# Lymphatus/caesium-clt

Hardware: AMD Instinct MI355X
Metric: megapixels/sec JPEG q=80 1920x1080 batch (higher is better)
Workload: dtype int32

## Files before the change

caesium-clt_amd/binding.py:

```python
import ctypes as C
import os

_HERE = os.path.dirname(os.path.abspath(__file__))
NPHASES = 8
NKERNELS = 36
PHASE_NAMES = ["decode", "pixel", "masks_flags_runs", "stats_tables", "sizes_scan", "pack", "stuff_assemble", "reserved"]


class CCSParameters(C.Structure):
    _fields_ = [("keep_metadata", C.c_bool), ("jpeg_quality", C.c_uint32), ("jpeg_chroma_subsampling", C.c_uint32),
                ("jpeg_progressive", C.c_bool), ("jpeg_optimize", C.c_bool), ("jpeg_preserve_icc", C.c_bool),
                ("png_quality", C.c_uint32), ("png_optimization_level", C.c_uint32), ("png_force_zopfli", C.c_bool),
                ("png_optimize", C.c_bool), ("gif_quality", C.c_uint32), ("webp_quality", C.c_uint32), ("webp_lossless", C.c_bool),
                ("tiff_compression", C.c_uint32), ("tiff_deflate_level", C.c_uint32), ("width", C.c_uint32), ("height", C.c_uint32)]


class CCSResult(C.Structure):
    _fields_ = [("success", C.c_bool), ("code", C.c_uint32), ("error_message", C.c_char_p)]


class CByteArray(C.Structure):
    _fields_ = [("data", C.POINTER(C.c_uint8)), ("length", C.c_size_t)]


class Timing(C.Structure):
    _fields_ = [("total_ms", C.c_float), ("phase_ms", C.c_float * NPHASES), ("kernel_ms", C.c_float * NKERNELS), ("in_bytes", C.c_uint64), ("out_bytes", C.c_uint64),
                ("pixels", C.c_uint64), ("coef_bytes", C.c_uint64), ("n_images", C.c_uint32), ("n_failed", C.c_uint32), ("n_seq_decoded", C.c_uint32), ("n_par_fallback", C.c_uint32), ("n_par_short", C.c_uint32), ("n_prog_decoded", C.c_uint32), ("n_refine_chains", C.c_uint32), ("n_search_extra", C.c_uint32), ("n_fused_lists", C.c_uint32), ("n_list_refine", C.c_uint32)]


class PngTiming(C.Structure):
    _fields_ = [("total_ms", C.c_float), ("kernel_ms", C.c_float * 16), ("in_bytes", C.c_uint64), ("out_bytes", C.c_uint64), ("pixels", C.c_uint64),
                ("raw_bytes", C.c_uint64), ("n_images", C.c_uint32), ("n_failed", C.c_uint32), ("n_trials", C.c_uint32)]


class CaesiumError(RuntimeError):
    def __init__(self, code, message):
        super().__init__(f"[{code}] {message}")
        self.code = code


def library_path():
    return os.path.join(_HERE, "libcaesium_hip.so")


EXPORTS = ["cs_default_parameters", "cs_compress_in_memory", "cs_compress_to_size_in_memory", "cs_convert_in_memory",
           "cs_batch_compress", "cs_batch_extent", "cs_free_bytes", "cs_free_result", "csh_device_count", "csh_last_error", "csh_kernel_name", "csh_kernel_name_webp", "csh_release_cached_memory", "csh_warmup", "csh_batch_create",
           "csh_batch_run", "csh_batch_fetch", "csh_batch_destroy", "csh_batch_retain_dct", "csh_batch_set_quality", "csh_batch_rerun_encode", "cs_batch_compress_to_size", "csh_batch_geometry", "csh_batch_read_coefs",
           "csp_kernel_name", "csp_batch_create", "csp_batch_create_webp", "csp_batch_create_pixels", "csh_batch_create_pixels", "csh_batch_pixels", "csh_batch_create_from_pixels", "csp_png_to_jpeg", "csp_png_to_lossless_webp", "csp_batch_run", "csp_batch_fetch", "csp_batch_destroy", "csp_batch_geometry", "csp_batch_read_rows", "csp_batch_read_stream",
           "csp_batch_trials", "csp_batch_read_scores", "csp_batch_chunk_bits", "csh_batch_create_webp", "cs_batch_convert",
           "cswd_batch_create", "cswd_batch_run", "cswd_batch_pixels", "cswd_batch_read_pixels", "cswd_batch_alpha", "cswd_batch_read_rgba", "cswd_batch_destroy", "cswd_rgba_join", "cswd_rgba_destroy", "csh_batch_create_webp_from_pixels", "csh_batch_create_from_pixels_rgb", "csl_encode_pixels", "csl_attach_alpha"]


def _declare(L):
    P = C.POINTER
    L.cs_default_parameters.argtypes = [P(CCSParameters)]
    L.cs_default_parameters.restype = None
    L.cs_compress_in_memory.argtypes = [C.c_char_p, C.c_size_t, P(CCSParameters), P(CByteArray)]
    L.cs_compress_in_memory.restype = CCSResult
    L.cs_compress_to_size_in_memory.argtypes = [C.c_char_p, C.c_size_t, P(CCSParameters), C.c_size_t, C.c_bool, P(CByteArray)]
    L.cs_compress_to_size_in_memory.restype = CCSResult
    L.cs_convert_in_memory.argtypes = [C.c_char_p, C.c_size_t, P(CCSParameters), C.c_uint32, P(CByteArray)]
    L.cs_convert_in_memory.restype = CCSResult
    L.cs_batch_compress.argtypes = [P(CByteArray), C.c_size_t, P(CCSParameters), C.c_int, P(CByteArray), P(CCSResult)]
    L.cs_batch_extent.argtypes = [P(CByteArray), C.c_size_t]
    L.cs_batch_extent.restype = C.c_size_t
    L.cs_free_bytes.argtypes = [P(CByteArray)]
    L.cs_free_bytes.restype = None
    L.cs_free_result.argtypes = [P(CCSResult)]
    L.cs_free_result.restype = None
    L.csh_last_error.restype = C.c_char_p
    L.csh_kernel_name.argtypes = [C.c_int]
    L.csh_kernel_name.restype = C.c_char_p
    L.csh_kernel_name_webp.argtypes = [C.c_int]
    L.csh_kernel_name_webp.restype = C.c_char_p
    L.csh_batch_create.argtypes = [P(CByteArray), C.c_size_t, P(CCSParameters), C.c_int, P(C.c_void_p)]
    L.csh_batch_run.argtypes = [C.c_void_p, P(Timing)]
    L.csh_batch_fetch.argtypes = [C.c_void_p, P(CByteArray), P(CCSResult)]
    L.csh_batch_retain_dct.argtypes = [C.c_void_p, C.c_int]
    L.csh_batch_set_quality.argtypes = [C.c_void_p, P(C.c_uint32)]
    L.csh_batch_rerun_encode.argtypes = [C.c_void_p, P(Timing)]
# ... 374 lines not shown
```

caesium-clt_amd/csrc/batch.hpp:

```cpp
#pragma once
#include <array>
#include <chrono>
#include <map>
#include <string>
#include <vector>

#include "../../include/caesium_hip.h"
#include "devmem.hpp"
#include "jpeg_host.hpp"
#include "kernels.h"
#include "webp_kernels.h"

namespace csh {

struct Item {
    int code = 0;
    std::string msg;
    JpegInfo in;
    JpegInfo out;
    int image = -1;
    size_t file_size = 0;
    std::vector<uint8_t> meta_out;
};

// ... 40 lines not shown
    uint32_t max_row_in = 0, max_out_w = 0, max_nh = 0;
    uint32_t max_src_px = 0;
    uint64_t plane_bytes = 0, oplane_bytes = 0;
    uint32_t max_quads = 0;
    bool any_layout = false, any_layout_rgb = false;

    DevBuf<uint8_t> d_planes, d_oplanes, d_rgb;
    DevBuf<PlaneWork> d_pwork;
    DevBuf<ResizeWork> d_rwork;
    DevBuf<ResizeTap> d_rtaps;
    DevBuf<float> d_rweights, d_rtmp;
    DevBuf<int16_t> d_dct_raw;
};

struct Stage {
    uint32_t work0 = 0, nwork = 0, slot0 = 0, nslots = 0, ech0 = 0, nech = 0, table0 = 0, ntables = 0, plan0 = 0, nplans = 0, nzc0 = 0, nnzc = 0, ls0 = 0, nls = 0, ts0 = 0, nts = 0, rs0 = 0, nrs = 0;
    bool nz_build[2] = {true, true}, nz_filter[2] = {true, true};
};
struct SearchImg {
    int cand_work[64]; int ncand;
    int Al_luma = 0, Al_chroma = 0;
    uint64_t best_luma = 0, best_chroma = 0;
    int split_luma = 0, split_chroma = 0;
    bool luma_on = false, chroma_on = false;
};

struct EncodePlan {
    std::vector<EncScan> script;
    std::vector<ScanWork> swork;
    uint32_t nslots = 0, nlist_slots = 0, ntok_slots = 0;
    uint32_t nref_slots = 0;
    uint32_t last_run_refine = 0;
    uint64_t total_corr = 0;
    uint64_t total_units = 0, total_words = 0;
    uint32_t max_units = 0;
    int ntables = 0;
    std::vector<TokPlan> plans;
    std::vector<int> plan_comp, plan_image;
    std::vector<EChunk> echunks;
    uint64_t tok_cap = 0;
    uint32_t tok_scale = 1;
    std::vector<TokRegion> regions;
    std::vector<uint32_t> region_est;
    uint32_t hist_rows = 0;
    std::vector<NzList> nzlists;
    std::vector<NzSet> nzsets;
    std::vector<int> nzset_of;
    std::vector<uint32_t> nzset_built;
    std::vector<int> nzset_comp, nzset_image;
    std::vector<NzChunk> nzchunks;
    std::vector<NzChunk> nzchunks_fused;
    uint32_t n_fused = 0;
    uint32_t last_run_fused = 0;
    std::vector<uint32_t> nz_est, nz_worst;
    uint32_t nz_nrec = 0;
    uint64_t nz_cap = 0;
    bool search = false;
    enum { ST_1 = 0, ST_1B = 1, ST_2 = 2, ST_2B = 3, ST_2C = 4, ST_N = 5 };
    Stage stage[ST_N];
    void stage_begin(Stage &sg) {
        sg.work0 = uint32_t(swork.size()); sg.slot0 = nslots; sg.ech0 = uint32_t(echunks.size()); sg.table0 = uint32_t(ntables); sg.plan0 = uint32_t(plans.size());
        sg.nzc0 = uint32_t(nzchunks.size()); sg.ls0 = nlist_slots; sg.ts0 = ntok_slots; sg.rs0 = nref_slots;
    }
    void stage_end(Stage &sg) {
        sg.nwork = uint32_t(swork.size()) - sg.work0; sg.nslots = nslots - sg.slot0; sg.nech = uint32_t(echunks.size()) - sg.ech0;
        sg.ntables = uint32_t(ntables) - sg.table0; sg.nplans = uint32_t(plans.size()) - sg.plan0;
        sg.nnzc = uint32_t(nzchunks.size()) - sg.nzc0; sg.nls = nlist_slots - sg.ls0; sg.nts = ntok_slots - sg.ts0; sg.nrs = nref_slots - sg.rs0;
    }
    std::vector<SearchImg> simg;
    std::vector<uint8_t> work_active;
    uint32_t n_gated_runs = 0;
    std::vector<uint32_t> img_list, img_nlist, h_cost;
    std::map<std::array<int, 5>, int> cand_script;
    std::vector<uint8_t> hdr_pool;
    std::vector<uint32_t> hdr_off;

    DevBuf<uint8_t> d_hdr, d_tail, d_scan_tmp, d_work_active;
    DevBuf<EncScan> d_script;
    DevBuf<ScanWork> d_swork;
    DevBuf<uint32_t> d_slot_work;
    DevBuf<EChunk> d_echunks;
    DevBuf<SlotRec> d_slots;
    DevBuf<TokPlan> d_plans;
    DevBuf<uint64_t> d_corr, d_symbits, d_eobbits, d_tok_off, d_chunk_off, d_scan_raw_off;
    DevBuf<uint32_t> d_tok_cursor;
    DevBuf<TokRegion> d_regions;
    DevBuf<uint16_t> d_eobrun, d_slot_hist;
    DevBuf<uint32_t> d_img_list, d_img_nlist, d_scan_cost, d_slot_raw, d_slot_eobh, d_long_runs, d_long_cnt, d_tokens, d_chunk_ntok, d_chunk_bits, d_raw, d_scan_pad, d_chunk_ff, d_hdr_off;
    DevBuf<DevEncTable> d_tables;
    DevBuf<NzList> d_nzlists;
    DevBuf<NzSet> d_nzsets;
    DevBuf<NzChunk> d_nzchunks, d_nzchunks_fused;
    DevBuf<uint32_t> d_nz_pool, d_nz_cursor, d_nz_chunk_off, d_nz_chunk_cnt, d_list_slots, d_tok_slots, d_ref_slots;
};

struct TrellisPlan {
    bool trellis = false, dering = false;
    Stage tstage;
    std::vector<TrellisWork> twork;
    std::vector<TrellisRun> truns;
    uint32_t t_units = 0, t_max_rows = 0;
    std::vector<uint32_t> trows;
    bool t_sort = false;
    bool nz_once = false;

    DevBuf<TrellisWork> d_twork;
// ... 50 lines not shown
    uint32_t ntiles = 0, ntiles_in = 0, ntiles_out = 0, max_tiles = 0, max_dummy = 0;
    csh::DevBuf<csh::ImgDesc> d_imgs;
    csh::DevBuf<csh::DevQuant> d_quants;
    csh::DevBuf<int16_t> d_coef;

    csh::DecodePlan dec;
    csh::PixelPlan pix;
    csh::EncodePlan enc;
    csh::TrellisPlan tr;
    csh::WebpTail wp;
    csh::Outputs out;

    ~csh_batch() { if (have_stream) { (void)hipStreamSynchronize(stream); (void)hipStreamDestroy(stream); } }
};

namespace csh {

enum KernelSlot {
    KS_MEMSET_COEF, KS_UNSTUFF, KS_DEC_SPEC, KS_DEC_RELAX0, KS_DEC_RELAX, KS_DEC_WRITE, KS_DC_SCATTER, KS_REFINE_CHAINS, KS_DECODE_PROG_SEQ,
    KS_IDCT_PLANE, KS_RESIZE, KS_XFORM_DIRECT, KS_RESAMPLE_FDCT, KS_FIX_DUMMY, KS_MEMSET_ENC, KS_TRELLIS_STATS, KS_TRELLIS_AC, KS_TRELLIS_DC,
    KS_NZLIST, KS_TOKENS, KS_LIST_STATS, KS_AC_RUNS, KS_GEN_TABLES, KS_CHUNK_SIZES, KS_SCAN_CHUNK_BITS, KS_SCAN_LAYOUT, KS_PACK, KS_LIST_PACK,
    KS_FF_COUNT, KS_SCAN_SEARCH, KS_LAYOUT, KS_SCAN_IMAGES, KS_EMIT, KS_SPARE0, KS_SPARE1, KS_SPARE2, KS_COUNT,
    KS_WEBP_YUV = KS_XFORM_DIRECT, KS_WEBP_ENCODE = KS_RESAMPLE_FDCT, KS_WEBP_ASSEMBLE = KS_FIX_DUMMY
};
struct KernelSlotRow { KernelSlot slot; const char *name; int phase; };
constexpr KernelSlotRow kKernelSlots[] = {
    {KS_MEMSET_COEF, "memset_coef", 0},        {KS_UNSTUFF, "unstuff", 0},                 {KS_DEC_SPEC, "k_dec_spec", 0},
    {KS_DEC_RELAX0, "k_dec_relax0", 0},        {KS_DEC_RELAX, "k_dec_relax1_4", 0},        {KS_DEC_WRITE, "k_dec_write", 0},
    {KS_DC_SCATTER, "k_dc_scatter", 0},        {KS_REFINE_CHAINS, "k_refine_chains", 0},   {KS_DECODE_PROG_SEQ, "k_decode_prog+seq", 0},
    {KS_IDCT_PLANE, "k_idct_plane", 1},        {KS_RESIZE, "resize", 1},                   {KS_XFORM_DIRECT, "k_xform_direct", 1},
    {KS_RESAMPLE_FDCT, "k_resample+k_plane_fdct", 1}, {KS_FIX_DUMMY, "k_fix_dummy", 1},    {KS_MEMSET_ENC, "memset_enc", 2},
    {KS_TRELLIS_STATS, "trellis_stats", 1},    {KS_TRELLIS_AC, "k_trellis_ac", 1},         {KS_TRELLIS_DC, "k_trellis_dc", 1},
    {KS_NZLIST, "k_nzlist", 2},                {KS_TOKENS, "k_tokens", 2},                 {KS_LIST_STATS, "k_list_stats", 2},
    {KS_AC_RUNS, "k_ac_runs", 2},              {KS_GEN_TABLES, "k_gen_tables", 3},         {KS_CHUNK_SIZES, "k_chunk_sizes", 4},
    {KS_SCAN_CHUNK_BITS, "scan_chunk_bits", 4}, {KS_SCAN_LAYOUT, "scan_layout", 4},        {KS_PACK, "k_pack", 5},
    {KS_LIST_PACK, "k_list_pack", 5},          {KS_FF_COUNT, "k_ff_count", 6},             {KS_SCAN_SEARCH, "scan_search_stage2", 7},
    {KS_LAYOUT, "k_layout", 6},                {KS_SCAN_IMAGES, "scan_images", 6},         {KS_EMIT, "k_emit", 6},
    {KS_SPARE0, "", 7},                        {KS_SPARE1, "", 7},                         {KS_SPARE2, "", 7}};
constexpr bool kernel_slots_in_order() {
    for (int i = 0; i < int(sizeof kKernelSlots / sizeof kKernelSlots[0]); i++) if (kKernelSlots[i].slot != i) return false;
    return true;
}
static_assert(sizeof kKernelSlots / sizeof kKernelSlots[0] == CSH_NKERNELS && int(KS_COUNT) == int(CSH_NKERNELS), "one row per csh_timing.kernel_ms slot");
static_assert(kernel_slots_in_order(), "row i of kKernelSlots describes slot i");

struct PlanSwitches {
    std::string profile;
    bool nz_once = true;
    bool tr_sort = true;
    int prog_par = -1;
    bool fused_420 = true;
    bool nz_fused = true;
    bool ref_list = true;
    static PlanSwitches read();
};

struct Laps {
    const bool trace;
    std::chrono::steady_clock::time_point at = std::chrono::steady_clock::now();
    std::string text;
    Laps();
    void lap(const char *what);
};

struct BatchPlanner {
    csh_batch *const b;
    const CByteArray *const inputs;
    const size_t count;
    const CCSParameters *const p;
    const csp_pixels *const px;
    const PlanSwitches sw;
    const bool progressive;
    uint16_t qout_nat[64];
    int script_base3 = 0, script_base1 = 0;
    std::vector<std::pair<std::vector<uint8_t>, int>> hset_keys;
    std::map<std::vector<uint16_t>, int> quant_index;
    uint64_t plane_off = 64, oplane_off = 0;

    BatchPlanner(csh_batch *b, const CByteArray *inputs, size_t count, const CCSParameters *p, const csp_pixels *px);
    void begin();
    void parse();
    int reserve_pinned();
    int plan_image(size_t n);
    int plan_search_stages();
    int plan_trellis();
    void finish_descriptors();
    int upload(Laps &laps);

private:
    void image_geometry(Item &it, ImgDesc &im);
    int decode_scans(Item &it, ImgDesc &im, const uint8_t *d);
    int huff_set(const JScan &js);
    void place_blocks(ParScan &ps, const JpegInfo &in, const JScan &js, uint32_t units, bool dc_rows, bool subseqs);
    int sequential_split(const Item &it, const ImgDesc &im, const uint8_t *d, int img_index, bool &par_ok);
    bool progressive_plan(const Item &it, const ImgDesc &im, int img_index);
    void plane_work(ImgDesc &im, const JpegInfo &in, const JpegInfo &o, int img_index, bool resized);
    void resize_work(const JpegInfo &in, const JpegInfo &o, int img_index);
    void output_scans(Item &it, ImgDesc &im, int img_index, size_t in_len);
    void frame_header(Item &it);
    template <class Fill> int enc_scan(const std::array<int, 5> &key, Fill fill);
    int cand_index(int comp, int Ss, int Se, int Ah, int Al);
    int dc_scan_index(int ncomp);
    int seq1_index(int comp);
    uint32_t nz_list(int img_index, int comp, int Al, const ImgDesc &im, size_t in_len);
    void add_works(Item &it, ImgDesc &im, int img_index, const std::vector<int> &list, size_t in_len, const JpegInfo &o, bool stats_only = false);
    template <class Make> void add_stage(int sid, Make make);
// ... 14 lines not shown
```

caesium-clt_amd/csrc/batch_plan.cpp:

```cpp
#include <algorithm>
#include <atomic>
#include <cmath>
#include <thread>

#include "batch.hpp"
#include "resize_host.h"

namespace csh {

static void build_dev_huff(const HuffSpec &h, DevHuff &d) {
    memset(&d, 0, sizeof d);
    for (int l = 0; l < 18; l++) d.maxcode[l] = -1;
    if (!h.present) return;
    int code = 0, p = 0;
    for (int l = 1; l <= 16; l++) {
        if (h.bits[l]) {
            d.valptr[l] = p - code;
            for (int i = 0; i < h.bits[l]; i++, p++, code++)
                if (l <= 9) {
                    int base = code << (9 - l);
                    for (int k = 0; k < (1 << (9 - l)); k++) d.look[(base + k) & 511] = uint16_t((l << 8) | h.vals[p]);
                }
            d.maxcode[l] = code - 1;
        }
// ... 140 lines not shown
        for (int c = 0; c < in.ncomp; c++) o.comp[c] = in.comp[c];
        jpeg_geometry(o);
        return 0;
    }
    int ss = int(p.jpeg_chroma_subsampling);
    if (ss == 0) ss = 420;
    for (int c = 0; c < in.ncomp; c++) { o.comp[c].id = c + 1; o.comp[c].h = o.comp[c].v = 1; o.comp[c].tq = c ? 1 : 0; }
    if (in.ncomp == 3) {
        int blocks = 0;
        for (int c = 0; c < 3; c++) {
            const JComp &k = in.comp[c];
            blocks += k.h * k.v;
            if (in.hmax % k.h || in.vmax % k.v) { it.msg = "fractional chroma sampling ratio (component factors do not divide the largest ones)"; return CS_ERR_JPEG_FEATURE; }
            if (in.hmax / k.h > 4 || in.vmax / k.v > 4) { it.msg = "chroma sampling ratio above 4"; return CS_ERR_JPEG_FEATURE; }
        }
        if (blocks > 10) { it.msg = "more than 10 blocks per MCU"; return CS_ERR_JPEG_FEATURE; }
        if (ss == 420) { o.comp[0].h = 2; o.comp[0].v = 2; }
        else if (ss == 422) { o.comp[0].h = 2; o.comp[0].v = 1; }
        else if (ss == 411) { o.comp[0].h = 4; o.comp[0].v = 1; }
        else if (ss != 444) { it.msg = "unknown output chroma subsampling"; return CS_ERR_JPEG_FEATURE; }
    }
    jpeg_geometry(o);
    return 0;
}

void layout_token_pool(csh_batch *b) {
    b->enc.regions.resize(b->enc.region_est.size());
    if (b->test_pool_shift < 0) b->test_pool_shift = getenv("CSH_TEST_POOL_SHIFT") ? std::min(16, std::max(0, atoi(getenv("CSH_TEST_POOL_SHIFT")))) : 0;
    const int shift = b->test_pool_shift;
    uint64_t at = 0;
    for (size_t i = 0; i < b->enc.regions.size(); i++) {
        const uint64_t cap = std::min<uint64_t>(std::max<uint64_t>((uint64_t(b->enc.region_est[i]) * b->enc.tok_scale) >> shift, 64), 0xFFFFFFF0ull);
        b->enc.regions[i].base = at; b->enc.regions[i].cap = uint32_t(cap); b->enc.regions[i].pad = 0;
        at += (cap + 3) & ~uint64_t(3);
    }
    b->enc.tok_cap = at + 64;
    at = 0;
    for (size_t i = 0; i < b->enc.nzlists.size(); i++) {
        const uint64_t cap = std::min<uint64_t>(std::max<uint64_t>((uint64_t(b->enc.nz_est[i]) * b->enc.tok_scale) >> shift, 64), b->enc.nz_worst[i]);
        b->enc.nzlists[i].base = at; b->enc.nzlists[i].cap = uint32_t(cap);
        at += (cap + 3) & ~uint64_t(3);
    }
    b->enc.nz_cap = at + 64;
}

PlanSwitches PlanSwitches::read() {
    auto is = [](const char *name, const char *v) { const char *e = getenv(name); return e && !strcmp(e, v); };
    PlanSwitches s;
    const char *penv = getenv("CSH_PROFILE");
    s.profile = penv && *penv ? penv : "mozjpeg";
    s.nz_once = !is("CSH_NZ_ONCE", "0");
    s.tr_sort = !is("CSH_TR_SORT", "0");
    s.nz_fused = !is("CSH_NZ_FUSED", "0");
    s.ref_list = is("CSH_REF_LIST", "1") || (s.ref_list && !is("CSH_REF_LIST", "0"));
    const char *pp = getenv("CSH_PROG_PAR");
    s.prog_par = pp && !strcmp(pp, "0") ? 0 : (pp && !strcmp(pp, "1") ? 1 : -1);
    s.fused_420 = !getenv("CSH_NO_FUSED_420");
    return s;
}

Laps::Laps() : trace(getenv("CSH_TRACE") != nullptr) {}
void Laps::lap(const char *what) {
    if (!trace) return;
    const auto now = std::chrono::steady_clock::now();
    char buf[64];
    snprintf(buf, sizeof buf, " %s %.1f", what, std::chrono::duration<double, std::milli>(now - at).count());
    text += buf; at = now;
}

BatchPlanner::BatchPlanner(csh_batch *b_, const CByteArray *inputs_, size_t count_, const CCSParameters *p_, const csp_pixels *px_)
    : b(b_), inputs(inputs_), count(count_), p(p_), px(px_), sw(PlanSwitches::read()), progressive(p_->jpeg_progressive) {}

void BatchPlanner::begin() {
    b->items.resize(count);
    quality_table(int(p->jpeg_quality), qout_nat);
    DevQuant qo; make_quant(qout_nat, qo);
    b->quants.push_back(qo);
    b->q_base = int(b->quants.size()) - 1;
    for (int q = 1; q <= 100; q++) { uint16_t tq[64]; quality_table(q, tq); DevQuant dq; make_quant(tq, dq); b->quants.push_back(dq); }
    b->progressive = progressive;

    add_script(b->enc.script, 3, true);
    add_script(b->enc.script, 1, true);
    add_script(b->enc.script, 3, false);
    add_script(b->enc.script, 1, false);
    script_base3 = progressive ? 0 : 16; script_base1 = progressive ? 10 : 17;
    const bool webp = b->webp, rgb_out = b->rgb_out;
    const std::string &profile = sw.profile;
    b->enc.search = progressive && !webp && !rgb_out && profile != "plain";
    const bool lossy_jpeg = !b->lossless && !webp && !rgb_out;
    b->tr.trellis = lossy_jpeg && (profile == "mozjpeg" || profile == "mozjpeg-trellis");
    b->tr.dering = lossy_jpeg && (profile == "mozjpeg" || profile == "mozjpeg-dering");
    b->tr.nz_once = b->tr.trellis && progressive && sw.nz_once && sw.tr_sort;
}

template <class Fill>
int BatchPlanner::enc_scan(const std::array<int, 5> &key, Fill fill) {
    auto f = b->enc.cand_script.find(key);
    if (f != b->enc.cand_script.end()) return f->second;
    EncScan e;
    memset(&e, 0, sizeof e);
    fill(e);
    b->enc.script.push_back(e);
    return b->enc.cand_script[key] = int(b->enc.script.size()) - 1;
}
int BatchPlanner::cand_index(int comp, int Ss, int Se, int Ah, int Al) {
// ... 391 lines not shown
bool BatchPlanner::progressive_plan(const Item &it, const ImgDesc &im, int img_index) {
    const JpegInfo &in = it.in;
    bool prog_ok = in.progressive && in.restart_interval == 0;
    for (size_t s = 0; s < in.scans.size(); s++) {
        const JScan &js = in.scans[s];
        if (js.has_marker || js.data_len >= (1u << 28) || !b->dec.phset_fits[b->dec.dscans[im.first_scan + s].huff_set]) prog_ok = false;
    }
    if (!prog_ok) return false;
    const bool par_first = regular_progression(in) && sw.prog_par != 0 && uint64_t(in.mcus_x) * uint64_t(in.mcus_y) * 10 < (1u << 24);
    for (size_t s = 0; s < in.scans.size(); s++) {
        const JScan &js = in.scans[s];
        DecScan &ds = b->dec.dscans[im.first_scan + s];
        ParScan ps;
        memset(&ps, 0, sizeof ps);
        ps.bits_off = ds.bits_off; ps.bits_len = ds.bits_len; ps.huff_set = ds.huff_set; ps.image = img_index; ps.ncomp = ds.ncomp; ps.nb_mcu = 1;
        ps.Ss = js.Ss; ps.Se = js.Se; ps.Al = js.Al;
        ps.kind = !par_first ? CSH_PS_UNSTUFF : js.Ss == 0 ? (js.Ah == 0 ? CSH_PS_DC_FIRST : CSH_PS_DC_REFINE) : (js.Ah == 0 ? CSH_PS_AC_FIRST : CSH_PS_UNSTUFF);
        ps.sub_base = b->dec.total_sub; ps.par_index = uint32_t(b->dec.pscans.size());
        if (ps.kind != CSH_PS_UNSTUFF) place_blocks(ps, in, js, scan_units(in, js), ps.kind == CSH_PS_DC_FIRST, ps.kind != CSH_PS_DC_REFINE);
        ds.par_index = int(b->dec.pscans.size());
        b->dec.pscans.push_back(ps);
    }
    const bool refine_split = par_first && sw.prog_par != 1;
    for (int chain = 0; chain <= in.ncomp; chain++) {
        ProgChain pc;
        memset(&pc, 0, sizeof pc);
        pc.image = img_index; pc.first = int(b->dec.chain_scans.size());
        bool all_refine = chain != 0;
        for (size_t s = 0; s < in.scans.size(); s++) {
            const JScan &js = in.scans[s];
            const bool mine = chain == 0 ? js.Ss == 0 : (js.Ss != 0 && js.comp_idx[0] == chain - 1);
            if (mine && b->dec.pscans[size_t(b->dec.dscans[im.first_scan + s].par_index)].kind == CSH_PS_UNSTUFF) {
                b->dec.chain_scans.push_back(im.first_scan + int(s)); pc.count++;
                if (js.Ah == 0 || js.data_len >= (1u << 27)) all_refine = false;
            }
        }
        if (pc.count && refine_split && all_refine) {
            const JComp &jc = in.comp[chain - 1];
            const uint64_t nblocks = uint64_t(jc.real_bw) * uint64_t(jc.real_bh);
            if (nblocks && uint64_t(b->dec.refine_pos) + nblocks * uint64_t(pc.count) < (1ull << 32)) {
                pc.refine = 1; pc.comp = chain - 1; pc.nblocks = uint32_t(nblocks);
                pc.hist_off = b->dec.refine_hist; pc.pos_off = b->dec.refine_pos;
                b->dec.refine_hist += pc.nblocks; b->dec.refine_pos += pc.nblocks * uint32_t(pc.count);
                b->dec.refine_max_blocks = std::max(b->dec.refine_max_blocks, pc.nblocks);
            }
        }
        if (pc.count) b->dec.chains.push_back(pc);
    }
    return true;
}

void BatchPlanner::plane_work(ImgDesc &im, const JpegInfo &in, const JpegInfo &o, int img_index, bool resized) {
    for (int c = 0; c < in.ncomp; c++) {
        PlaneWork w; w.image = img_index; w.comp = c; w.nzset = 0xFFFFFFFFu;
        w.up = resized ? up_desc(1, 1, 0) : up_desc(in.hmax / in.comp[c].h, in.vmax / in.comp[c].v, in.comp[c].comp_w);
        w.dn = dn_kind(o.hmax / o.comp[c].h, o.vmax / o.comp[c].v);
        const int in_kind = (w.up.hx == 1 && w.up.vx == 1) ? 0 : (w.up.hx == 2 && w.up.vx == 2) ? 1 : (w.up.hx == 2 && w.up.vx == 1) ? 2 : -1;
        if (in_kind < 0 || w.dn == CSH_DN_H4V1) w.mode = CSH_MODE_ANY;
        else if (resized) w.mode = 1 + w.dn;
        else w.mode = (in_kind == 0 && w.dn == CSH_DN_FULL) ? 0 : 1 + 3 * in_kind + w.dn;
        if (w.mode == CSH_MODE_ANY) b->pix.any_layout = true;
        const bool fused = w.mode == 5 && !resized && im.in[c].comp_w > 2 && im.in[c].real_bw == im.out[c].real_bw && im.in[c].real_bh == im.out[c].real_bh &&
                           im.in[c].comp_w == im.out[c].comp_w && im.in[c].comp_h == im.out[c].comp_h && sw.fused_420;
        if (fused) w.mode = 10;
        if (w.mode) {
            im.plane_off[c] = plane_off;
            plane_off += uint64_t(im.in[c].real_bw * 8) * uint64_t(im.in[c].real_bh * 8);
            plane_off = (plane_off + 63u) & ~uint64_t(63);
            im.splane_off[c] = im.plane_off[c];
            if (resized) {
                JComp full; full.h = full.v = 1;
                JpegInfo tmpj; tmpj.width = o.width; tmpj.height = o.height; tmpj.ncomp = 1; tmpj.comp[0] = full; jpeg_geometry(tmpj);
                uint32_t dummy = 0; fill_geom(tmpj.comp[0], im.src[c], dummy);
                im.splane_off[c] = plane_off;
                plane_off += uint64_t(im.src[c].real_bw * 8) * uint64_t(im.src[c].real_bh * 8);
                plane_off = (plane_off + 63u) & ~uint64_t(63);
            }
            im.oplane_off[c] = oplane_off;
            const uint64_t osz = fused ? 0 : uint64_t(im.out[c].real_bw) * 8 * uint64_t(im.out[c].real_bh) * 8;
            oplane_off = (oplane_off + osz + 63u) & ~uint64_t(63);
            b->pix.max_quads = std::max(b->pix.max_quads, uint32_t(osz / 4));
        }
        b->pix.pwork.push_back(w);
    }
}

void BatchPlanner::resize_work(const JpegInfo &in, const JpegInfo &o, int img_index) {
    ResizeWork rw;
    memset(&rw, 0, sizeof rw);
    rw.image = img_index; rw.nw = o.width; rw.nh = o.height;
    rw.in_kind = in.ncomp == 1 ? 0 : ((in.comp[1].h == in.hmax && in.comp[1].v == in.vmax) ? 0 : (in.comp[1].v == in.vmax ? 2 : 1));
    for (int c = 0; c < in.ncomp; c++) rw.up[c] = up_desc(in.hmax / in.comp[c].h, in.vmax / in.comp[c].v, in.comp[c].comp_w);
    if (in.ncomp == 3) {
        auto same = [&](int c, int hx, int vx) { return rw.up[c].hx == hx && rw.up[c].vx == vx; };
        const bool legacy = same(0, 1, 1) && rw.up[1].hx == rw.up[2].hx && rw.up[1].vx == rw.up[2].vx &&
                            (same(1, 1, 1) || same(1, 2, 2) || same(1, 2, 1));
        if (!legacy) { rw.in_kind = CSH_RZ_ANY; b->pix.any_layout_rgb = true; }
    }
    if (px) rw.in_kind = -1;
    const uint64_t src_bytes = uint64_t(in.width) * in.height * in.ncomp, dst_bytes = uint64_t(o.width) * o.height * in.ncomp;
    rw.rgb_src_off = b->pix.rgb_bytes; b->pix.rgb_bytes += (src_bytes + 63) & ~uint64_t(63);
    rw.rgb_dst_off = b->pix.rgb_bytes; b->pix.rgb_bytes += (dst_bytes + 63) & ~uint64_t(63);
    const uint64_t tmpn = uint64_t(o.height) * in.width * in.ncomp;
    rw.tmp_off = b->pix.tmp_floats; b->pix.tmp_floats += tmpn;
    const bool same = o.width == in.width && o.height == in.height;
    rw.vtap_base = uint32_t(b->pix.rtaps.size()); csh_lanczos_axis(in.height, o.height, same, b->pix.rtaps, b->pix.rweights);
    rw.htap_base = uint32_t(b->pix.rtaps.size()); csh_lanczos_axis(in.width, o.width, same, b->pix.rtaps, b->pix.rweights);
// ... 168 lines not shown
        const size_t first = b->enc.swork.size();
        add_works(it, im, it.image, list, inputs[n].length, it.out, true);
        for (int c = 0; c < im.ncomp; c++) {
            const ScanWork &w = b->enc.swork[first + size_t(c)];
            TrellisWork tw;
            memset(&tw, 0, sizeof tw);
            tw.image = it.image; tw.comp = c;
            tw.table_ac = w.table_base + (progressive ? 0u : 1u);
            tw.table_dc = progressive ? -1 : int32_t(w.table_base);
            tw.nunits = w.nunits; tw.unit_base = b->tr.t_units;
            b->tr.t_units += w.nunits;
            b->tr.t_max_rows = std::max<uint32_t>(b->tr.t_max_rows, uint32_t((im.out[c].real_bh + im.out[c].v - 1) / im.out[c].v));
            tw.nzset = 0xFFFFFFFFu;
            if (progressive) {
                const int si = b->enc.nzset_of[size_t(it.image) * CSH_MAX_COMPS + size_t(c)];
                b->enc.nzsets[size_t(si)].cnt_base = tw.unit_base;
                if (b->tr.nz_once) tw.nzset = uint32_t(si);
            }
            b->tr.twork.push_back(tw);
        }
    }
    b->enc.stage_end(tg);
    {
        std::vector<uint32_t> nch(b->tr.twork.size());
        uint32_t most = 0;
        for (size_t wi = 0; wi < b->tr.twork.size(); wi++) { nch[wi] = (b->tr.twork[wi].nunits + CSH_TR_WG - 1) / CSH_TR_WG; most = std::max(most, nch[wi]); }
        for (uint32_t j = 0; j < most; j += CSH_TR_RUN)
            for (size_t wi = 0; wi < b->tr.twork.size(); wi++)
                if (j < nch[wi]) b->tr.truns.push_back(TrellisRun{uint32_t(wi), j, std::min<uint32_t>(CSH_TR_RUN, nch[wi] - j)});
    }
    {
        b->tr.t_sort = progressive && sw.tr_sort;
        std::vector<std::pair<uint32_t, uint32_t>> rows;
        for (size_t wi = 0; wi < b->tr.twork.size(); wi++) {
            const CompGeom &g = b->imgs[size_t(b->tr.twork[wi].image)].out[b->tr.twork[wi].comp];
            for (int r = 0; r < (g.real_bh + g.v - 1) / g.v; r++) rows.push_back({uint32_t(g.real_bw * g.v), uint32_t(wi << 16) | uint32_t(r)});
        }
        std::stable_sort(rows.begin(), rows.end(), [](const auto &a, const auto &b2) { return a.first > b2.first; });
        for (const auto &r : rows) b->tr.trows.push_back(r.second);
    }
    if (b->enc.total_units > 0xFFFFFFF0ull) { csh_set_error("csh_batch_create: batch too large (fewer files per batch)"); return CS_ERR_POOL_OVERFLOW; }
    return 0;
}

void BatchPlanner::finish_descriptors() {
    if (!b->lossless)
        for (ImgDesc &im : b->imgs) for (int c = 0; c < im.ncomp; c++) im.out[c].tile_base += b->ntiles_in;
    for (size_t i = 0; i < b->enc.plans.size(); i++) b->enc.plans[i].tile_base = b->imgs[size_t(b->enc.plan_image[i])].out[b->enc.plan_comp[i]].tile_base;
    for (size_t i = 0; i < b->enc.nzsets.size(); i++) b->enc.nzsets[i].tile_base = b->imgs[size_t(b->enc.nzset_image[i])].out[b->enc.nzset_comp[i]].tile_base;
    {
        b->enc.nzchunks_fused = b->enc.nzchunks;
        const bool allowed = sw.nz_fused && !b->lossless && !b->webp && !b->rgb_out && !(b->tr.trellis && progressive && !b->tr.nz_once);
        std::vector<uint8_t> fused(b->enc.nzsets.size(), 0);
        for (PlaneWork &w : b->pix.pwork) {
            const size_t at = size_t(w.image) * CSH_MAX_COMPS + size_t(w.comp);
            const int si = allowed && at < b->enc.nzset_of.size() ? b->enc.nzset_of[at] : -1;
            if (si < 0) continue;
            const NzSet &S = b->enc.nzsets[size_t(si)];
            if (S.real_bw != S.bw || S.list[0] == 0xFFFFFFFFu) continue;
            w.nzset = uint32_t(si); fused[size_t(si)] = 1; b->enc.n_fused++;
        }
        for (NzChunk &ch : b->enc.nzchunks_fused) if (fused[ch.set]) ch.levels &= ~1u;
        auto flags = [&](Stage &sg) {
            for (int f = 0; f < 2; f++) {
                const std::vector<NzChunk> &v = f ? b->enc.nzchunks_fused : b->enc.nzchunks;
                sg.nz_build[f] = sg.nz_filter[f] = false;
                for (uint32_t i = sg.nzc0; i < sg.nzc0 + sg.nnzc; i++) { sg.nz_build[f] |= (v[i].levels & 1u) != 0u; sg.nz_filter[f] |= (v[i].levels & ~1u) != 0u; }
            }
        };
        for (Stage &sg : b->enc.stage) flags(sg);
        flags(b->tr.tstage);
    }
    for (ParScan &ps : b->dec.pscans)
        for (int m = 0; m < ps.nb_mcu && m < 10; m++) {
            int dcs = ps.dct[m] & 3, acs = 4 + (ps.act[m] & 3);
            if (b->dec.use4) { dcs = std::max<int>(0, b->dec.slot4[ps.huff_set][dcs]); acs = std::max<int>(0, b->dec.slot4[ps.huff_set][acs]); }
            ps.sel |= uint64_t(dcs | (acs << 3)) << (6 * m);
        }
    {
        std::vector<int> last(b->dec.chains.size(), -1);
        for (int s = 0;; s++) {
            bool any = false;
            for (size_t c = 0; c < b->dec.chains.size(); c++)
                if (b->dec.chains[c].refine && b->dec.chains[c].count > s) {
                    RefineUnit u; u.chain = int(c); u.s = s; u.prev = last[c];
                    last[c] = int(b->dec.refine_units.size());
                    b->dec.refine_units.push_back(u);
                    any = true;
                }
            if (!any) break;
        }
    }
    b->ntiles = b->ntiles_in + b->ntiles_out;
    b->pix.plane_bytes = plane_off;
    b->pix.oplane_bytes = oplane_off;
    b->out.out_cap = b->out.raw_bytes_cap;
    layout_token_pool(b);
}

int BatchPlanner::upload(Laps &laps) {
    hipStream_t st = b->stream;
    if (!b->nimg) return 0;
    b->dec.bits_pool.flush_copies();
    laps.lap("copy_in");
    if (b->dec.d_bits.alloc(b->dec.bits_pool.size()) || (b->dec.bits_pool.size() && hipMemcpyAsync(b->dec.d_bits.p, b->dec.bits_pool.p, b->dec.bits_pool.size(), hipMemcpyHostToDevice, st) != hipSuccess) ||
        b->d_imgs.upload(b->imgs, st) || b->dec.d_dscans.upload(b->dec.dscans, st) || b->dec.d_chains.upload(b->dec.chains, st) || b->dec.d_chain_scans.upload(b->dec.chain_scans, st) ||
        b->dec.d_hsets.upload(b->dec.hsets, st) || b->dec.d_phsets.upload(b->dec.phsets, st) || (b->dec.use4 && b->dec.d_phsets4.upload(b->dec.phsets4, st)) || b->d_quants.upload(b->quants, st) || b->pix.d_pwork.upload(b->pix.pwork, st) ||
        b->enc.d_script.upload(b->enc.script, st) || b->enc.d_swork.upload(b->enc.swork, st) || b->enc.d_slot_work.alloc(size_t(b->enc.nslots) + 1) || b->enc.d_slots.alloc(size_t(b->enc.nslots) + 1) || b->enc.d_plans.upload(b->enc.plans, st) || b->enc.d_echunks.upload(b->enc.echunks, st) || b->enc.d_hdr.upload(b->enc.hdr_pool, st) ||
        b->enc.d_hdr_off.upload(b->enc.hdr_off, st) || b->dec.d_pscans.upload(b->dec.pscans, st) || b->pix.d_rwork.upload(b->pix.rwork, st) || b->pix.d_rtaps.upload(b->pix.rtaps, st) ||
        b->pix.d_rweights.upload(b->pix.rweights, st) || b->pix.d_rgb.alloc(b->pix.rgb_bytes + 64) || b->pix.d_rtmp.alloc((resize_is_fused(b->pix.max_row_in) ? 0 : b->pix.tmp_floats) + 16) || b->dec.d_need_seq_init.upload(b->dec.need_seq_init, st))
        return CS_ERR_NO_DEVICE;
    size_t nchunks = b->dec.bits_pool.size() / 64 + 1, nst = size_t(b->dec.total_sub) + b->dec.pscans.size() + 1;
    if (b->dec.d_clean.alloc(b->dec.bits_pool.size() + 64) || b->dec.d_unstuff_cnt.alloc(nchunks + 1) || b->dec.d_unstuff_off.alloc(nchunks + 2) ||
        b->dec.d_pstate.alloc(nst) || b->dec.d_relax_list[0].alloc(nst) || b->dec.d_relax_list[1].alloc(nst) || b->dec.d_relax_cnt.alloc(512) || b->dec.d_scan_pending.alloc(b->dec.pscans.size() + 1) || b->dec.d_cut_block.alloc(b->dec.pscans.size() + 1) || b->dec.d_claim.alloc(size_t(b->dec.total_sub) + 1) || b->dec.d_hyp.alloc((size_t(b->dec.total_sub) + 1) * 10) ||
// ... 38 lines not shown
```

caesium-clt_amd/csrc/batch_run.cpp:

```cpp
#include <algorithm>

#include "batch.hpp"

namespace csh {
namespace {

class KernelMarks {
    hipEvent_t ev[CSH_NKERNELS + 1];
    int created = 0, next = 0;
    const hipStream_t st;

public:
    explicit KernelMarks(hipStream_t s) : st(s) {}
    KernelMarks(const KernelMarks &) = delete;
    KernelMarks &operator=(const KernelMarks &) = delete;
    ~KernelMarks() { for (int i = 0; i < created; i++) (void)hipEventDestroy(ev[i]); }
    int start() {
        for (; created <= CSH_NKERNELS; created++) CSH_CHECK(hipEventCreate(&ev[created]));
        CSH_CHECK(hipEventRecord(ev[0], st));
        return 0;
    }
    int claim(KernelSlot slot, hipEvent_t *e) {
        if (int(slot) != next || next >= CSH_NKERNELS) {
            csh_set_error("internal: timing mark '%s' out of order (slot %d is next)", slot < KS_COUNT ? kKernelSlots[slot].name : "?", next);
// ... 113 lines not shown
                uint32_t left = 0;
                CSH_CHECK(hipMemcpyAsync(&left, b->dec.d_relax_cnt.p + R, sizeof left, hipMemcpyDeviceToHost, st));
                CSH_CHECK(hipStreamSynchronize(st));
                if (!left) break;
            }
            if (nps) {
                if (b->dec.d_scan_pending.zero(st)) return -1;
                launch_dec_mark_pending(st, b->dec.d_pscans.p, b->dec.total_sub, b->dec.d_relax_list[R & 1].p, b->dec.d_relax_cnt.p + R, b->dec.d_scan_pending.p);
                da.hyp = b->dec.d_hyp.p; da.scan_pending = b->dec.d_scan_pending.p;
                launch_dec_dense(st, 3, nps, b->dec.max_sub, da);
                launch_dec_chain(st, b->dec.d_pscans.p, nps, b->dec.d_pstate.p, b->dec.d_nblk.p, b->dec.d_hyp.p, b->dec.d_scan_pending.p, b->dec.d_need_seq.p);
            }
            MARK(KS_DEC_RELAX);
            if (nps) launch_exclusive_scan(st, b->dec.d_nblk.p, b->dec.d_blk_off.p, b->dec.total_sub, b->enc.d_scan_tmp.p, b->enc.d_scan_tmp.n);
            launch_dec_dense(st, 2, nps, b->dec.max_sub, da);
            MARK(KS_DEC_WRITE);
            if (nps) launch_exclusive_scan(st, reinterpret_cast<uint32_t *>(b->dec.d_dcdiff.p), b->dec.d_dc_off.p, b->dec.dc_total, b->enc.d_scan_tmp.p, b->enc.d_scan_tmp.n);
            launch_dc_scatter(st, b->dec.d_pscans.p, nps, b->dec.max_par_blocks, b->d_imgs.p, b->dec.d_dc_off.p, b->d_coef.p, b->dec.d_need_seq.p, b->dec.d_cut_block.p);
            launch_dc_refine(st, b->dec.d_clean.p, b->dec.d_pscans.p, nps, b->dec.max_par_blocks, b->d_imgs.p, b->d_coef.p, b->dec.d_need_seq.p);
            MARK(KS_DC_SCATTER);
        }
        launch_refine_chains(st, b->dec.d_clean.p, b->dec.d_pscans.p, b->dec.d_phsets.p, b->dec.d_dscans.p, b->dec.d_chains.p, b->dec.d_chain_scans.p, int(b->dec.chains.size()), b->dec.d_refine_units.p,
                             int(b->dec.refine_units.size()), b->dec.refine_max_blocks, b->d_imgs.p, b->d_coef.p, b->dec.d_need_seq.p, b->dec.d_refine_hist.p, b->dec.d_refine_pos.p, b->dec.d_refine_prog.p);
        MARK(KS_REFINE_CHAINS);
        launch_decode_prog(st, b->dec.d_clean.p, b->dec.d_pscans.p, b->dec.d_phsets.p, b->dec.d_dscans.p, b->dec.d_chains.p, b->dec.d_chain_scans.p, int(b->dec.chains.size()), b->d_imgs.p,
                           b->d_coef.p, b->dec.d_need_seq.p);
        launch_decode_seq(st, b->dec.d_bits.p, b->d_imgs.p, b->dec.d_dscans.p, b->dec.d_hsets.p, b->d_coef.p, nimg, b->dec.d_need_seq.p);
        MARK(KS_DECODE_PROG_SEQ);
        return 0;
    }

    int planes() {
        int nw = b->lossless ? 0 : int(b->pix.pwork.size());
        launch_idct_plane(st, b->d_imgs.p, b->pix.d_pwork.p, nw, b->max_tiles, b->d_quants.p, b->d_coef.p, b->pix.d_planes.p);
        MARK(KS_IDCT_PLANE);
        launch_resize(st, b->d_imgs.p, b->pix.d_rwork.p, int(b->pix.rwork.size()), b->pix.d_rtaps.p, b->pix.d_rweights.p, b->pix.d_planes.p, b->pix.d_rgb.p, b->pix.d_rtmp.p,
                      b->pix.max_src_px, b->pix.max_tmp, b->pix.max_dst, b->pix.max_row_in, b->pix.max_out_w, b->pix.max_nh, !(b->webp || b->rgb_out), b->pix.any_layout_rgb);
        MARK(KS_RESIZE);
        return 0;
    }
    int pixels() {
        const int nw = b->lossless ? 0 : int(b->pix.pwork.size());
        int16_t *rawp = ((b->retain_dct || b->tr.trellis) && !b->lossless) ? b->pix.d_dct_raw.p : nullptr;
        NzFuse nzf;
        memset(&nzf, 0, sizeof nzf);
        fused = nw && b->enc.n_fused;
        if (fused) {
            if (b->enc.d_nz_cursor.zero(st) || b->enc.d_nz_chunk_cnt.zero(st)) return -1;
            nzf.nzsets = b->enc.d_nzsets.p; nzf.nzlists = b->enc.d_nzlists.p; nzf.nz_pool = b->enc.d_nz_pool.p; nzf.nz_cursor = b->enc.d_nz_cursor.p;
            nzf.nz_chunk_off = b->enc.d_nz_chunk_off.p; nzf.nz_chunk_cnt = b->enc.d_nz_chunk_cnt.p; nzf.overflow = b->out.d_overflow.p;
            nzf.blk_cnt = (b->tr.trellis && b->tr.t_sort) ? b->tr.d_tblk_cnt.p : nullptr;
            nzf.blk_off = (nzf.blk_cnt && b->tr.nz_once) ? b->tr.d_tblk_off.p : nullptr;
        }
        launch_xform_direct(st, b->d_imgs.p, b->pix.d_pwork.p, nw, b->max_tiles, b->d_quants.p, b->d_coef.p, b->d_coef.p, rawp, b->ntiles_in, b->tr.dering, nzf);
        MARK(KS_XFORM_DIRECT);
        launch_resample_plane(st, b->d_imgs.p, b->pix.d_pwork.p, nw, b->pix.max_quads, b->pix.d_planes.p, b->pix.d_oplanes.p);
        if (b->pix.any_layout) launch_resample_any(st, b->d_imgs.p, b->pix.d_pwork.p, nw, b->pix.max_quads, b->pix.d_planes.p, b->pix.d_oplanes.p);
        launch_plane_fdct(st, b->d_imgs.p, b->pix.d_pwork.p, nw, b->max_tiles, b->d_quants.p, b->pix.d_oplanes.p, b->d_coef.p, rawp, b->ntiles_in, b->tr.dering, nzf);
        launch_resample_fdct_420(st, b->d_imgs.p, b->pix.d_pwork.p, nw, b->max_tiles, b->d_quants.p, b->pix.d_planes.p, b->d_coef.p, rawp, b->ntiles_in, b->tr.dering, nzf);
        MARK(KS_RESAMPLE_FDCT);
        if (!b->lossless) launch_fix_dummy(st, b->d_imgs.p, nimg, b->max_dummy, b->d_coef.p);
        MARK(KS_FIX_DUMMY);
        return 0;
    }

    void fill_enc_ctx() {
        memset(&c, 0, sizeof c);
        c.imgs = b->d_imgs.p; c.script = b->enc.d_script.p; c.work = b->enc.d_swork.p; c.nwork = int(b->enc.swork.size());
        c.echunks = b->enc.d_echunks.p; c.plans = b->enc.d_plans.p; c.nechunks = uint32_t(b->enc.echunks.size()); c.slot_work = b->enc.d_slot_work.p; c.slots = b->enc.d_slots.p; c.nslots = b->enc.nslots;
        c.coef = b->d_coef.p; c.sym_bits = b->enc.d_symbits.p; c.eob_bits = b->enc.d_eobbits.p; c.tail = b->enc.d_tail.p;
        c.eobrun = b->enc.d_eobrun.p; c.long_runs = b->enc.d_long_runs.p; c.long_cnt = b->enc.d_long_cnt.p; c.corr = b->enc.d_corr.p;
        c.tokens = b->enc.d_tokens.p; c.regions = b->enc.d_regions.p; c.tok_cursor = b->enc.d_tok_cursor.p; c.tok_off = b->enc.d_tok_off.p; c.chunk_ntok = b->enc.d_chunk_ntok.p; c.slot_hist = b->enc.d_slot_hist.p; c.slot_raw = b->enc.d_slot_raw.p; c.slot_eobh = b->enc.d_slot_eobh.p;
        c.chunk_bits = b->enc.d_chunk_bits.p; c.chunk_off = b->enc.d_chunk_off.p; c.tables = b->enc.d_tables.p;
        c.raw = b->enc.d_raw.p; c.raw_words = raw_chunks * 16; c.status = b->out.d_status.p; c.overflow = b->out.d_overflow.p;
        c.nzlists = b->enc.d_nzlists.p; c.nzsets = b->enc.d_nzsets.p; c.nz_pool = b->enc.d_nz_pool.p; c.nz_cursor = b->enc.d_nz_cursor.p; c.nz_chunk_off = b->enc.d_nz_chunk_off.p; c.nz_chunk_cnt = b->enc.d_nz_chunk_cnt.p;
        c.debug = getenv("CSH_DEBUG") ? uint32_t(atoi(getenv("CSH_DEBUG"))) : 0u;
    }
    void fill_asm_ctx() {
        memset(&a, 0, sizeof a);
        a.imgs = b->d_imgs.p; a.script = b->enc.d_script.p; a.work = b->enc.d_swork.p; a.nimg = nimg;
        a.nwork = b->tr.trellis ? int(b->tr.tstage.work0) : c.nwork;
        a.tables = b->enc.d_tables.p; a.chunk_off = b->enc.d_chunk_off.p; a.scan_pad_bytes = b->enc.d_scan_pad.p; a.scan_raw_off = b->enc.d_scan_raw_off.p;
        a.raw = b->enc.d_raw.p; a.raw_chunks = raw_chunks; a.chunk_ff = b->enc.d_chunk_ff.p;
        a.hdr_pool = b->enc.d_hdr.p; a.hdr_off = b->enc.d_hdr_off.p; a.img_size = b->out.d_img_size.p; a.img_size_pad = b->out.d_img_size_pad.p;
        a.img_off = b->out.d_img_off.p; a.out = b->out.d_out.p; a.out_cap = b->out.out_cap; a.status = b->out.d_status.p; a.overflow = b->out.d_overflow.p;
        a.img_list = b->enc.d_img_list.p; a.img_nlist = b->enc.d_img_nlist.p; a.scan_cost = b->enc.d_scan_cost.p;
    }
    void fill_trellis_ctx(TrellisCtx &tc) {
        memset(&tc, 0, sizeof tc);
        tc.imgs = b->d_imgs.p; tc.quant = b->d_quants.p; tc.work = b->tr.d_twork.p; tc.nwork = int(b->tr.twork.size()); tc.runs = b->tr.d_truns.p; tc.nruns = uint32_t(b->tr.truns.size());
        tc.tables = b->enc.d_tables.p; tc.raw = b->pix.d_dct_raw.p; tc.raw_tile0 = b->ntiles_in; tc.coef = b->d_coef.p; tc.dcrec = b->tr.d_tlambda.p; tc.dcbt = b->tr.d_tdcbt.p;
        tc.spill = b->tr.d_tspill.p; tc.nslots = uint32_t(b->tr.d_tspill.n / trellis_spill_words(1)); tc.max_rows = b->tr.t_max_rows;
        tc.queue = b->tr.d_tqueue.p;
        tc.rows = b->tr.d_trows.p; tc.nrows = uint32_t(b->tr.trows.size());
        if (b->tr.t_sort) { tc.blk_cnt = b->tr.d_tblk_cnt.p; tc.perm = b->tr.d_tperm.p; }
        if (b->tr.t_sort && b->tr.nz_once) {
            tc.nz_pool = b->enc.d_nz_pool.p; tc.nzlists = b->enc.d_nzlists.p; tc.nzsets = b->enc.d_nzsets.p; tc.nz_chunk_off = b->enc.d_nz_chunk_off.p; tc.nz_chunk_cnt = b->enc.d_nz_chunk_cnt.p;
            tc.blk_off = b->tr.d_tblk_off.p;
        }
        tc.debug = getenv("CSH_TR_DEBUG") ? uint32_t(atoi(getenv("CSH_TR_DEBUG"))) : 0u;
    }

    int encode_begin() {
        fill_enc_ctx();
        launch_reset_works(st, b->enc.d_swork.p, c.nwork);
        if (!fused && (b->enc.d_nz_cursor.zero(st) || b->enc.d_nz_chunk_cnt.zero(st))) return -1;
        if (b->enc.d_symbits.zero(st) || b->enc.d_eobbits.zero(st) || (!eobrun_cleared && b->enc.d_eobrun.zero(st)) || b->enc.d_tables.zero(st) || b->enc.d_tok_cursor.zero(st) || b->enc.d_slot_eobh.zero(st) || b->enc.d_scan_pad.zero(st)) return -1;
#ifdef CSH_EMUL
        if (b->enc.d_raw.zero(st)) return -1;
#else
        if ((c.debug & 8192u) && b->enc.d_raw.zero(st)) return -1;
#endif
        MARK(KS_MEMSET_ENC);
        return 0;
    }

    void set_stage(const Stage &sg) {
        c.echunks = b->enc.d_echunks.p + sg.ech0; c.nechunks = sg.nech; c.slot0 = sg.slot0; c.nslots = sg.nslots;
        c.nzchunks = (fused ? b->enc.d_nzchunks_fused.p : b->enc.d_nzchunks.p) + sg.nzc0; c.nnzchunks = sg.nnzc;
        c.nz_build = sg.nz_build[fused ? 1 : 0]; c.nz_filter = sg.nz_filter[fused ? 1 : 0];
        c.list_slots = b->enc.d_list_slots.p + sg.ls0; c.nlist_slots = sg.nls; c.tok_slots = b->enc.d_tok_slots.p + sg.ts0; c.ntok_slots = sg.nts;
        c.ref_slots = b->enc.d_ref_slots.p + sg.rs0; c.nref_slots = sg.nrs;
    }

    int trellis() {
        const Stage &tg = b->tr.tstage;
        set_stage(tg);
        c.stats_only = 1;
        if (b->enc.d_long_cnt.zero(st)) return -1;
        c.nz_blk_cnt = b->tr.t_sort ? b->tr.d_tblk_cnt.p : nullptr;
        c.nz_blk_off = (b->tr.t_sort && b->tr.nz_once) ? b->tr.d_tblk_off.p : nullptr;
        launch_nzlist(st, c);
        c.nz_blk_cnt = nullptr; c.nz_blk_off = nullptr;
        if (b->tr.t_sort) {
            TrellisCtx ts;
            memset(&ts, 0, sizeof ts);
            ts.work = b->tr.d_twork.p; ts.nwork = int(b->tr.twork.size()); ts.blk_cnt = b->tr.d_tblk_cnt.p; ts.perm = b->tr.d_tperm.p;
            launch_trellis_sort(st, ts);
        }
        launch_tokens(st, c);
        launch_list_stats(st, c);
        launch_ac_runs(st, c);
        launch_gen_tables(st, b->enc.d_tables.p + tg.table0, int(tg.ntables));
        c.stats_only = 0;
        if (b->enc.d_nz_cursor.zero(st)) return -1;
        MARK(KS_TRELLIS_STATS);
        TrellisCtx tc;
        fill_trellis_ctx(tc);
        if (b->tr.d_tqueue.zero(st)) return -1;
        launch_trellis_ac(st, tc);
        MARK(KS_TRELLIS_AC);
        launch_trellis_dc(st, tc);
// ... 65 lines not shown
        MARK(KS_LAYOUT);
        launch_exclusive_scan(st, b->out.d_img_size_pad.p, b->out.d_img_off.p, uint64_t(nimg), b->enc.d_scan_tmp.p, b->enc.d_scan_tmp.n);
        MARK(KS_SCAN_IMAGES);
        launch_emit(st, a);
        MARK(KS_EMIT);
        return 0;
    }

    int finish(bool phases) {
        CSH_CHECK(hipStreamSynchronize(st));
        CSH_CHECK(hipGetLastError());
        if (t && marks.read(t, phases)) return -1;
        if (t && !phases) t->n_images = uint32_t(nimg);
        return 0;
    }

    int webp() {
        const int nwimg = int(b->wp.wimgs.size());
        uint64_t out_bytes = 0;
        std::vector<uint64_t> off(size_t(b->nimg) + 1, 0);
        for (auto &wi : b->wp.wimgs) {
            const uint64_t cap = 4096 + uint64_t(wi.mbw) * wi.mbh * (b->wp.webp_mb_bytes + 2);
            wi.out_cap = uint32_t(std::min<uint64_t>(cap, 0xFFFFFF00u)); wi.out_off = out_bytes;
            off[wi.image] = out_bytes;
            out_bytes += (wi.out_cap + 63) & ~uint64_t(63);
            const int q = int(b->params.webp_quality);
            wi.quality = q < 0 ? 0 : q > 100 ? 100 : q;
        }
        off[b->nimg] = out_bytes;
        if (b->out.d_out.n < out_bytes + 64 && b->out.d_out.alloc(out_bytes + 64)) return -1;
        if ((b->wp.d_wscratch.n < out_bytes + 64 && b->wp.d_wscratch.alloc(out_bytes + 64)) || (b->wp.d_wpart.n < size_t(b->nimg) * 9 + 9 && b->wp.d_wpart.alloc(size_t(b->nimg) * 9 + 9)) ||
            (b->wp.d_wstats.n < size_t(b->nimg) * 2112 + 8 && (b->wp.d_wstats.alloc(size_t(b->nimg) * 2112 + 8) || b->wp.d_wprobs.alloc(size_t(b->nimg) * 1056 + 8) || b->wp.d_wupdate.alloc(size_t(b->nimg) * 1056 + 8))))
            return -1;
        if (b->wp.d_wstats.zero(st)) return -1;
        if (b->wp.d_wimgs.upload(b->wp.wimgs, st) || (b->wp.d_wwork.n < b->wp.wwork_bytes + 64 && b->wp.d_wwork.alloc(b->wp.wwork_bytes + 64)) ||
            (b->wp.d_wlevels.n < b->wp.wlevels + 64 && b->wp.d_wlevels.alloc(b->wp.wlevels + 64)))
            return -1;
        CSH_CHECK(hipMemcpyAsync(b->out.d_img_off.p, off.data(), off.size() * sizeof(uint64_t), hipMemcpyHostToDevice, st));
        if (b->out.d_img_size.zero(st)) return -1;
        csw::launch_webp_yuv(st, b->wp.d_wimgs.p, nwimg, b->wp.wmax_luma, b->pix.d_rgb.p, b->wp.d_wwork.p);
        MARK(KS_WEBP_YUV);
        hipEvent_t mid;
        if (marks.claim(KS_WEBP_ENCODE, &mid)) return -1;
        if (csw::launch_webp_encode(st, b->wp.wimgs.data(), nwimg, b->wp.d_wimgs.p, b->wp.d_wwork.p, b->wp.d_wlevels.p, b->wp.d_wscratch.p, b->wp.d_wpart.p, b->out.d_out.p, b->out.d_img_size.p, b->out.d_status.p, mid)) return -1;
        MARK(KS_WEBP_ASSEMBLE);
        return finish(false);
    }
};

}

int run_once(csh_batch *b, csh_timing *t, bool requant_only) {
    Run r(b, t);
    b->enc.last_run_fused = 0; b->enc.last_run_refine = 0;
    if (r.pools() || r.marks.start()) return -1;
    const bool from_pixels = requant_only && b->tr.dering;
    if (requant_only && !from_pixels) {
        if (r.requant()) return -1;
    } else {
        if (from_pixels ? r.skip_decode() : r.decode()) return -1;
        if (r.planes()) return -1;
        if (b->webp) return r.webp();
        if (b->rgb_out) return (r.marks.mark(KS_XFORM_DIRECT) || r.finish(false)) ? -1 : 0;
        if (r.pixels()) return -1;
    }
    if (r.encode_begin()) return -1;
    b->enc.last_run_fused = r.fused ? b->enc.n_fused : 0u;
    if (b->tr.trellis ? r.trellis() : r.marks.skip_to(KS_NZLIST)) return -1;
    r.fill_asm_ctx();
    if (r.stage(b->enc.stage[0], true, false)) return -1;
    if (b->enc.search && r.search()) return -1;
    return (r.emit() || r.finish(true)) ? -1 : 0;
}

}
```

caesium-clt_amd/csrc/k_aclist.hip:

```cpp
#include "kernels.h"
#include "wave.h"

namespace csh {

#define CSH_LP_WORDS 1024

__device__ __forceinline__ static uint32_t lbitlen(uint32_t v) { return 32u - uint32_t(__clz(v)); }
__device__ __forceinline__ static int lwave() { return int(threadIdx.x) / CSP_WAVE_THREADS; }

#define CSH_NZ_HALF 16
__device__ __forceinline__ static uint4 nz_load(const EncCtx &c, const NzSet &S, uint32_t u, int bx, int by, uint32_t oct) {
    uint4 q; q.x = q.y = q.z = q.w = 0u;
    if (u < S.nunits) {
        const int b = by * S.bw + bx;
        q = *reinterpret_cast<const uint4 *>(c.coef + (size_t(S.tile_base) + size_t(b >> 6)) * CSH_TILE_I16 + size_t((b & 63) * CSH_BLK_STRIDE) + size_t(oct) * CSH_OCT_STRIDE);
    }
    return q;
}
__device__ __forceinline__ static uint32_t nz_mask8(const uint4 &q, uint32_t oct) {
    uint32_t m = 0;
    m |= (q.x & 0xFFFFu) ? 1u : 0u;   m |= (q.x >> 16) ? 2u : 0u;
    m |= (q.y & 0xFFFFu) ? 4u : 0u;   m |= (q.y >> 16) ? 8u : 0u;
    m |= (q.z & 0xFFFFu) ? 16u : 0u;  m |= (q.z >> 16) ? 32u : 0u;
    m |= (q.w & 0xFFFFu) ? 64u : 0u;  m |= (q.w >> 16) ? 128u : 0u;
// ... 134 lines not shown
    uint32_t n0new = n0;
    dstL[0] = nullptr; runL[0] = 0; okL[0] = false;
    if (compact0 && n0) {
        dstL[0] = c.nz_pool + L0.base + c.nz_chunk_off[L0.chunk0 + ch.j];
        okL[0] = true;
        n0new = lsum32(cntL[0]);
    }
    for (int L = 1; L < CSH_NZ_LEVELS; L++) {
        dstL[L] = nullptr; runL[L] = 0; okL[L] = false;
        if (!((others >> L) & 1u)) continue;
        const NzList LL = c.nzlists[S.list[L]];
        const uint32_t n = lsum32(cntL[L]), na = (n + 3u) & ~3u;
        uint32_t rel = 0;
        LFOR(l) if (l == 0) rel = atomicAdd(&c.nz_cursor[S.list[L]], na);
        rel = uni(rel);
        okL[L] = n0 != 0u && uint64_t(rel) + na <= LL.cap;
        dstL[L] = c.nz_pool + LL.base + rel;
        LFOR(l) {
            if (l == 0) { c.nz_chunk_off[LL.chunk0 + ch.j] = rel; c.nz_chunk_cnt[LL.chunk0 + ch.j] = okL[L] ? n : 0u; if (!okL[L]) c.overflow[1] = 1; }
            if (okL[L] && n + uint32_t(l) < na) dstL[L][n + uint32_t(l)] = 0u;
        }
    }
    for (uint32_t g0 = 0; g0 < n0; g0 += 256) {
        LV<uint32_t> e0, e1, e2, e3;
        LFOR(l) {
            const uint32_t g = g0 + 4u * uint32_t(l);
            uint4 e; e.x = e.y = e.z = e.w = 0u;
            if (g < n0) e = *reinterpret_cast<const uint4 *>(src + g);
            e0[l] = e.x; e1[l] = e.y; e2[l] = e.z; e3[l] = e.w;
        }
        for (int L = Lfirst; L < CSH_NZ_LEVELS; L++) {
            if (!okL[L]) continue;
            LV<uint32_t> k4;
            LFOR(l) k4[l] = kept(e0[l], L) + kept(e1[l], L) + kept(e2[l], L) + kept(e3[l], L);
            uint32_t tot;
            const LV<uint32_t> ex = lscan(k4, tot);
            LFOR(l) {
                const uint32_t e[4] = {e0[l], e1[l], e2[l], e3[l]};
                uint32_t o = runL[L] + ex[l];
                CSH_UNROLL
                for (int q = 0; q < 4; q++)
                    if (kept(e[q], L)) dstL[L][o++] = (e[q] & 0xFF8000FFu) | ((((e[q] >> 8) & 0x7FFFu) >> L) << 8);
            }
            runL[L] += tot;
        }
    }
    if (okL[0]) {
        const uint32_t na = (n0new + 3u) & ~3u;
        LFOR(l) {
            if (n0new + uint32_t(l) < na) dstL[0][n0new + uint32_t(l)] = 0u;
            if (l == 0) c.nz_chunk_cnt[L0.chunk0 + ch.j] = n0new;
        }
    }
}

struct NzEvent { uint32_t coded, term, run, size, bits, has, eob, blk; };
__device__ __forceinline__ static NzEvent nz_event(uint32_t e, uint32_t p, uint32_t Ss, uint32_t Se) {
    NzEvent v;
    const uint32_t k = e & 127u, pk = p & 127u;
    const bool same = !(p & CSH_NZ_END);
    const bool pin = same && pk >= Ss;
    v.coded = (k >= Ss && k <= Se) ? 1u : 0u;
    v.term = (k > Se && !(same && pk > Se)) ? 1u : 0u;
    v.run = k - (pin ? pk + 1u : Ss);
    const uint32_t m = (e >> 8) & 0x7FFFu;
    v.size = lbitlen(m);
    v.bits = ((e & 128u) ? ~m : m) & ((1u << v.size) - 1u);
    v.has = pin ? 1u : 0u;
    v.eob = (pin && pk == Se) ? 0u : 1u;
    v.blk = (e >> 23) & 255u;
    return v;
}
struct ListSlot { const uint32_t *lst; uint32_t n; };
__device__ __forceinline__ static ListSlot list_of_slot(const EncCtx &c, const SlotRec &r) {
    ListSlot s;
    s.n = c.nz_chunk_cnt[r.nzrec];
    s.lst = c.nz_pool + c.nzlists[r.nzlist].base + c.nz_chunk_off[r.nzrec];
    return s;
}
__device__ __forceinline__ static void list_load4(const ListSlot &s, uint32_t g, uint32_t &e0, uint32_t &e1, uint32_t &e2, uint32_t &e3) {
    uint4 q; q.x = q.y = q.z = q.w = 0u;
    if (g < s.n) q = *reinterpret_cast<const uint4 *>(s.lst + g);
    e0 = q.x; e1 = q.y; e2 = q.z; e3 = q.w;
}

__global__ void __launch_bounds__(256) k_list_stats(EncCtx c) {
    CSH_SHARED uint32_t s_hist[4][4][256];
    CSH_SHARED uint32_t s_flag[4][16];
    const int wv = lwave();
    const uint32_t idx = blockIdx.x * 4u + uint32_t(wv);
    if (idx >= c.nlist_slots) return;
    const uint32_t cs = c.list_slots[idx];
    const SlotRec r = c.slots[cs];
    if (c.work_active && !c.work_active[r.work]) return;
    const ListSlot ls = list_of_slot(c, r);
    uint32_t *hist = &s_hist[wv][0][0], *flag = s_flag[wv];
    LFOR(l) { for (int i = l; i < 1024; i += 64) hist[i] = 0u; if (l < 16) flag[l] = 0u; }
    CSP_WAVE_SYNC();
    const uint32_t Ss = r.Ss, Se = r.Se;
    uint32_t carry = CSH_NZ_END;
    LV<uint32_t> raw;
    LFOR(l) raw[l] = 0u;
    LV<uint32_t> x0, x1, x2, x3;
    LFOR(l) list_load4(ls, 4u * uint32_t(l), x0[l], x1[l], x2[l], x3[l]);
    for (uint32_t g0 = 0; g0 < ls.n; g0 += 256) {
        const LV<uint32_t> e0 = x0, e1 = x1, e2 = x2, e3 = x3;
// ... 395 lines not shown
```

caesium-clt_amd/csrc/k_pixel.hip:

```cpp
#include <cmath>
#include <utility>

#include "kernels.h"
#ifndef CSH_EMUL
#include "wave.h"
#endif

namespace csh {

static constexpr uint8_t kZ2N[64] = {0,  1,  8,  16, 9,  2,  3,  10, 17, 24, 32, 25, 18, 11, 4,  5,  12, 19, 26, 33, 40, 48,
                                     41, 34, 27, 20, 13, 6,  7,  14, 21, 28, 35, 42, 49, 56, 57, 50, 43, 36, 29, 22, 15, 23,
                                     30, 37, 44, 51, 58, 59, 52, 45, 38, 31, 39, 46, 53, 60, 61, 54, 47, 55, 62, 63};
template <int I>
__device__ __forceinline__ static int half_of(const uint4 &v) {
    uint32_t w = (I / 2 == 0) ? v.x : (I / 2 == 1) ? v.y : (I / 2 == 2) ? v.z : v.w;
    return (I & 1) ? (int(w) >> 16) : (int(w << 16) >> 16);
}
using Oct = std::integer_sequence<int, 0, 1, 2, 3, 4, 5, 6, 7>;
#ifndef CSH_EMUL
typedef uint32_t nt_u32x4 __attribute__((ext_vector_type(4)));
__device__ __forceinline__ static void nt_store16(void *p, const uint4 &v) { nt_u32x4 x; x.x = v.x; x.y = v.y; x.z = v.z; x.w = v.w; __builtin_nontemporal_store(x, reinterpret_cast<nt_u32x4 *>(p)); }
__device__ __forceinline__ static uint4 nt_load16(const void *p) { const nt_u32x4 x = __builtin_nontemporal_load(reinterpret_cast<const nt_u32x4 *>(p)); uint4 v; v.x = x.x; v.y = x.y; v.z = x.z; v.w = x.w; return v; }
#else
__device__ __forceinline__ static void nt_store16(void *p, const uint4 &v) { *reinterpret_cast<uint4 *>(p) = v; }
// ... 63 lines not shown
    return __builtin_amdgcn_perm(hi, lo, 0x05040100u);
#endif
}
__device__ __forceinline__ static uint32_t float_bits(float f) { uint32_t u; __builtin_memcpy(&u, &f, 4); return u; }

template <int J, int... I>
__device__ __forceinline__ static void dequant_octet(int x[64], const uint4 &v, const DevQuant &q, std::integer_sequence<int, I...>) {
    ((x[kZ2N[8 * J + I]] = MUL(half_of<I>(v), int(q.q[8 * J + I]))), ...);
}
template <int... J>
__device__ __forceinline__ static void load_dequant(const int16_t *__restrict__ blk, const DevQuant &q, int x[64], std::integer_sequence<int, J...>) {
    const uint4 v[8] = {nt_load16(blk + CSH_OCT_STRIDE * J)...};
    (dequant_octet<J>(x, v[J], q, Oct()), ...);
}
template <bool CENTRED = false>
__device__ __forceinline__ static void load_idct(const int16_t *__restrict__ blk, const DevQuant &q, int x[64]) {
    load_dequant(blk, q, x, Oct());
    CSH_SCHED_FENCE();
    CSH_UNROLL
    for (int c = 0; c < 8; c++) idct1d<11>(x[c], x[8 + c], x[16 + c], x[24 + c], x[32 + c], x[40 + c], x[48 + c], x[56 + c]);
    CSH_SCHED_FENCE();
    CSH_UNROLL
    for (int r = 0; r < 8; r++) {
        idct1d<18>(x[8 * r], x[8 * r + 1], x[8 * r + 2], x[8 * r + 3], x[8 * r + 4], x[8 * r + 5], x[8 * r + 6], x[8 * r + 7]);
        CSH_UNROLL
        for (int c = 0; c < 8; c++) {
            if (CENTRED) { const int v = x[8 * r + c]; x[8 * r + c] = v < -128 ? -128 : (v > 127 ? 127 : v); }
            else { const int v = x[8 * r + c] + 128; x[8 * r + c] = v < 0 ? 0 : (v > 255 ? 255 : v); }
        }
    }
    CSH_SCHED_FENCE();
}

__device__ __forceinline__ static void replicate_edges(int x[64], int vc, int vr) {
    CSH_UNROLL
    for (int c = 1; c < 8; c++) {
        const bool keep = c < vc;
        CSH_UNROLL
        for (int r = 0; r < 8; r++) x[8 * r + c] = keep ? x[8 * r + c] : x[8 * r + c - 1];
    }
    CSH_UNROLL
    for (int r = 1; r < 8; r++) {
        const bool keep = r < vr;
        CSH_UNROLL
        for (int c = 0; c < 8; c++) x[8 * r + c] = keep ? x[8 * r + c] : x[8 * (r - 1) + c];
    }
}

template <int K>
__device__ __forceinline__ static uint32_t quant_one(const int x[64], const DevQuant &q) {
    return float_bits(__builtin_fmaf(float(x[kZ2N[K]]), q.rcp[K], 12582912.0f));
}
template <int J>
__device__ __forceinline__ static void quant_store_octet(const int x[64], const DevQuant &q, int16_t *__restrict__ blk , uint4 &v) {
    v.x = pack_halves(quant_one<8 * J + 0>(x, q), quant_one<8 * J + 1>(x, q));
    v.y = pack_halves(quant_one<8 * J + 2>(x, q), quant_one<8 * J + 3>(x, q));
    v.z = pack_halves(quant_one<8 * J + 4>(x, q), quant_one<8 * J + 5>(x, q));
    v.w = pack_halves(quant_one<8 * J + 6>(x, q), quant_one<8 * J + 7>(x, q));
    nt_store16(blk + CSH_OCT_STRIDE * (J & 3), v);
}
template <int... J>
__device__ __forceinline__ static void quant_store_all(const int x[64], const DevQuant &q, int16_t *__restrict__ blk, uint4 lv[8], std::integer_sequence<int, J...>) {
    int16_t *hi = blk + 4 * CSH_OCT_STRIDE;
#ifndef CSH_EMUL
    asm volatile("" : "+v"(hi));
#endif
    ((quant_store_octet<J>(x, q, J < 4 ? blk : hi, lv[J]), CSH_SCHED_FENCE()), ...);
}
template <int J>
__device__ __forceinline__ static void raw_store_octet(const int x[64], int16_t *__restrict__ raw) {
    uint4 v;
    v.x = pack_halves(uint32_t(x[kZ2N[8 * J + 0]]), uint32_t(x[kZ2N[8 * J + 1]]));
    v.y = pack_halves(uint32_t(x[kZ2N[8 * J + 2]]), uint32_t(x[kZ2N[8 * J + 3]]));
    v.z = pack_halves(uint32_t(x[kZ2N[8 * J + 4]]), uint32_t(x[kZ2N[8 * J + 5]]));
    v.w = pack_halves(uint32_t(x[kZ2N[8 * J + 6]]), uint32_t(x[kZ2N[8 * J + 7]]));
    *reinterpret_cast<uint4 *>(raw + CSH_RAW_OCT * J) = v;
}
template <int... J>
__device__ __forceinline__ static void raw_store_all(const int x[64], int16_t *__restrict__ raw, std::integer_sequence<int, J...>) {
    (raw_store_octet<J>(x, raw), ...);
}
#ifdef CSH_EMUL
#define CSH_RAW_VIA_LDS 0
#else
#define CSH_RAW_VIA_LDS 1
#endif
template <int J>
__device__ __forceinline__ static void raw_put_octet(const int x[64], int16_t (*tr)[256], int tid) {
    uint4 v;
    v.x = pack_halves(uint32_t(x[kZ2N[8 * J + 0]]), uint32_t(x[kZ2N[8 * J + 1]]));
    v.y = pack_halves(uint32_t(x[kZ2N[8 * J + 2]]), uint32_t(x[kZ2N[8 * J + 3]]));
    v.z = pack_halves(uint32_t(x[kZ2N[8 * J + 4]]), uint32_t(x[kZ2N[8 * J + 5]]));
    v.w = pack_halves(uint32_t(x[kZ2N[8 * J + 6]]), uint32_t(x[kZ2N[8 * J + 7]]));
    const int l = tid & 63;
    *reinterpret_cast<uint4 *>(&tr[l][(tid & ~63) + 8 * (J ^ (l & 7))]) = v;
}
template <int... J>
__device__ __forceinline__ static void raw_put_all(const int x[64], int16_t (*tr)[256], int tid, std::integer_sequence<int, J...>) {
    (raw_put_octet<J>(x, tr, tid), ...);
}
__device__ __forceinline__ static void raw_copy_out(int16_t *__restrict__ tile_raw, bool has_raw, int16_t (*tr)[256], int tid) {
#if CSH_RAW_VIA_LDS
    const uint64_t mask = __ballot(has_raw);
    if (!mask) return;
    __builtin_amdgcn_fence(__ATOMIC_ACQ_REL, "wavefront");
    __builtin_amdgcn_wave_barrier();
    const int l = tid & 63;
    CSH_UNROLL
    for (int j = 0; j < 8; j++) {
        const int src = 8 * j + (l >> 3);
        if ((mask >> src) & 1ull) {
            const uint4 v = *reinterpret_cast<const uint4 *>(&tr[src][(tid & ~63) + 8 * ((l & 7) ^ (src & 7))]);
            nt_store16(tile_raw + src * 64 + (l & 7) * CSH_RAW_OCT, v);
        }
    }
#else
    (void)tile_raw; (void)has_raw; (void)tr; (void)tid;
#endif
}
#define CSH_DERING_LDS int16_t (*dr_col)[256]
// ... 75 lines not shown
#ifdef CSH_EMUL
    o0 = dot2(P, KE0P, dot2(Q, KE0Q, R0)); o4 = dot2(P, KE4P, dot2(Q, KE4Q, R4));
    o2 = dot2(P, KE2P, dot2(Q, KE2Q, R)); o6 = dot2(P, KE6P, dot2(Q, KE6Q, R));
    o7 = dot2(M, PK(kO7[3], kO7[2]), dot2(N, PK(kO7[1], kO7[0]), R));
    o5 = dot2(M, PK(kO5[3], kO5[2]), dot2(N, PK(kO5[1], kO5[0]), R));
    o3 = dot2(M, PK(kO3[3], kO3[2]), dot2(N, PK(kO3[1], kO3[0]), R));
    o1 = dot2(M, PK(kO1[3], kO1[2]), dot2(N, PK(kO1[1], kO1[0]), R));
#else
    asm("v_dot2_i32_i16 %0, %5, %8, %11\n\tv_dot2_i32_i16 %1, %5, %10, %12\n\tv_dot2_i32_i16 %2, %5, %14, %7\n\tv_dot2_i32_i16 %3, %5, %16, %7\n\t"
        "v_dot2_i32_i16 %0, %4, %6, %0\n\tv_dot2_i32_i16 %1, %4, %9, %1\n\tv_dot2_i32_i16 %2, %4, %13, %2\n\tv_dot2_i32_i16 %3, %4, %15, %3\n\ts_nop 2"
        : "=&v"(o0), "=&v"(o4), "=&v"(o2), "=&v"(o6)
        : "v"(P), "v"(Q), "s"(KE0P), "v"(R), "s"(KE0Q), "s"(KE4P), "s"(KE4Q), "v"(R0), "v"(R4), "s"(KE2P), "s"(KE2Q), "s"(KE6P), "s"(KE6Q));
    asm("v_dot2_i32_i16 %0, %5, %8, %6\n\tv_dot2_i32_i16 %1, %5, %10, %6\n\tv_dot2_i32_i16 %2, %5, %12, %6\n\tv_dot2_i32_i16 %3, %5, %14, %6\n\t"
        "v_dot2_i32_i16 %0, %4, %7, %0\n\tv_dot2_i32_i16 %1, %4, %9, %1\n\tv_dot2_i32_i16 %2, %4, %11, %2\n\tv_dot2_i32_i16 %3, %4, %13, %3\n\ts_nop 2"
        : "=&v"(o7), "=&v"(o5), "=&v"(o3), "=&v"(o1)
        : "v"(M), "v"(N), "v"(R), "s"(PK(kO7[3], kO7[2])), "s"(PK(kO7[1], kO7[0])), "s"(PK(kO5[3], kO5[2])), "s"(PK(kO5[1], kO5[0])),
          "s"(PK(kO3[3], kO3[2])), "s"(PK(kO3[1], kO3[0])), "s"(PK(kO1[3], kO1[2])), "s"(PK(kO1[1], kO1[0])));
#endif
    if (!FIRST) { o0 >>= 2; o4 >>= 2; }
    o2 >>= SH; o6 >>= SH; o7 >>= SH; o5 >>= SH; o3 >>= SH; o1 >>= SH;
}
template <bool CENTRED>
__device__ __forceinline__ static void dering_block_pk(uint32_t pr[8][4], int dc_quant, CSH_DERING_LDS) {
    uint32_t m = pr[0][0];
    CSH_UNROLL
    for (int i = 1; i < 32; i++) m = pk_max(m, pr[i >> 2][i & 3]);
    const int top = CENTRED ? 127 : 255, off = CENTRED ? 0 : 128;
    const bool any = int(int16_t(m)) >= top || int(int16_t(m >> 16)) >= top;
#ifndef CSH_EMUL
    if (!__ballot(any)) return;
#endif
    if (!any) return;
    int x[64];
    CSH_UNROLL
    for (int r = 0; r < 8; r++) {
        const uint32_t A = pr[r][0], B = pr[r][1], C = pr[r][2], D = pr[r][3];
        x[8 * r + 0] = int(int16_t(A)) - off; x[8 * r + 1] = int(int16_t(A >> 16)) - off; x[8 * r + 2] = int(int16_t(C)) - off; x[8 * r + 3] = int(int16_t(C >> 16)) - off;
        x[8 * r + 4] = int(int16_t(D >> 16)) - off; x[8 * r + 5] = int(int16_t(D)) - off; x[8 * r + 6] = int(int16_t(B >> 16)) - off; x[8 * r + 7] = int(int16_t(B)) - off;
    }
    int cnt = 0, sum = 0;
    CSH_UNROLL
    for (int i = 0; i < 64; i++) { sum += x[i]; cnt += x[i] >= 127 ? 1 : 0; }
    if (cnt == 64) return;
    int16_t *col = &dr_col[0][threadIdx.x];
    CSH_UNROLL
    for (int i = 0; i < 64; i++) col[i * 256] = int16_t(x[i]);
    dering_walk(col, dc_quant, cnt, sum);
    CSH_UNROLL
    for (int r = 0; r < 8; r++) {
        auto at = [&](int c) { return uint32_t(int(col[(8 * r + c) * 256]) + off); };
        pr[r][0] = pack_halves(at(0), at(1)); pr[r][1] = pack_halves(at(7), at(6)); pr[r][2] = pack_halves(at(2), at(3)); pr[r][3] = pack_halves(at(5), at(4));
    }
}
struct BlkOut { int16_t *coef_out; uint32_t tile_base; int b; int16_t *dct_raw; uint32_t raw_tile_base; };
template <bool DERING, bool CENTRED>
__device__ __forceinline__ static void fdct_quant_store_pk(uint32_t pr[8][4], const DevQuant &q, const BlkOut &o, uint4 lv[8], CSH_DERING_LDS) {
    CSH_SCHED_FENCE();
    if (DERING) { dering_block_pk<CENTRED>(pr, int(q.q[0]), dr_col); CSH_SCHED_FENCE(); }
    int x[64];
    int R = 1 << 10, Z = 0;
    CSH_PIN(R); CSH_PIN(Z);
    CSH_UNROLL
    for (int r = 0; r < 8; r++)
        fdct1d_pk<true>(pr[r][0], pr[r][1], pr[r][2], pr[r][3], R, Z, Z, x[8 * r], x[8 * r + 1], x[8 * r + 2], x[8 * r + 3], x[8 * r + 4], x[8 * r + 5], x[8 * r + 6], x[8 * r + 7]);
    CSH_SCHED_FENCE();
    int R2 = 1 << 14, TWO = 2, RDC = 2 - 32768;
    CSH_PIN(R2); CSH_PIN(TWO); CSH_PIN(RDC);
    CSH_UNROLL
    for (int c = 0; c < 8; c++) {
        const uint32_t A = pack_halves(uint32_t(x[c]), uint32_t(x[8 + c])), B = pack_halves(uint32_t(x[56 + c]), uint32_t(x[48 + c]));
        const uint32_t C = pack_halves(uint32_t(x[16 + c]), uint32_t(x[24 + c])), D = pack_halves(uint32_t(x[40 + c]), uint32_t(x[32 + c]));
        fdct1d_pk<false>(A, B, C, D, R2, (c == 0 && !CENTRED) ? RDC : TWO, TWO, x[c], x[8 + c], x[16 + c], x[24 + c], x[32 + c], x[40 + c], x[48 + c], x[56 + c]);
    }
    CSH_SCHED_FENCE();
    int b = o.b;
    CSH_PIN(b);
    if (o.dct_raw) {
        if (CSH_RAW_VIA_LDS) raw_put_all(x, dr_col, int(threadIdx.x), Oct()); else raw_store_all(x, o.dct_raw + raw_index(o.raw_tile_base, b), Oct());
    }
    quant_store_all(x, q, o.coef_out + coef_index(o.tile_base, b, 0), lv, Oct());
}
__device__ __forceinline__ static void pack_rows(const int x[64], uint32_t pr[8][4]) {
    CSH_UNROLL
    for (int r = 0; r < 8; r++) {
        pr[r][0] = pack_halves(uint32_t(x[8 * r]), uint32_t(x[8 * r + 1])); pr[r][1] = pack_halves(uint32_t(x[8 * r + 7]), uint32_t(x[8 * r + 6]));
        pr[r][2] = pack_halves(uint32_t(x[8 * r + 2]), uint32_t(x[8 * r + 3])); pr[r][3] = pack_halves(uint32_t(x[8 * r + 5]), uint32_t(x[8 * r + 4]));
    }
}
template <bool DERING, bool CENTRED = false>
__device__ __forceinline__ static void fdct_quant_store(int x[64], const DevQuant &q, const BlkOut &o, uint4 lv[8], CSH_DERING_LDS) {
    uint32_t pr[8][4];
    pack_rows(x, pr);
    fdct_quant_store_pk<DERING, CENTRED>(pr, q, o, lv, dr_col);
}
template <bool DERING, bool CENTRED = false>
__device__ __forceinline__ static void fdct_quant_store(int x[64], const DevQuant &q, int16_t *__restrict__ blk, int16_t *__restrict__ raw, CSH_DERING_LDS) {
    uint4 lv[8];
    fdct_quant_store<DERING, CENTRED>(x, q, BlkOut{blk, 0u, 0, raw, 0u}, lv, dr_col);
}

template <int J, int... I>
__device__ __forceinline__ static void raw_to_nat(int x[64], const uint4 &v, std::integer_sequence<int, I...>) {
    ((x[kZ2N[8 * J + I]] = half_of<I>(v)), ...);
}
template <int... J>
__device__ __forceinline__ static void requant_block(const int16_t *__restrict__ raw, const DevQuant &q, int16_t *__restrict__ blk, std::integer_sequence<int, J...>) {
    const uint4 v[8] = {*reinterpret_cast<const uint4 *>(raw + CSH_RAW_OCT * J)...};
    int x[64];
    (raw_to_nat<J>(x, v[J], Oct()), ...);
    uint4 lv[8];
    quant_store_all(x, q, blk, lv, Oct());
}

__device__ __forceinline__ static void store_zero_block(int16_t *__restrict__ blk) {
    uint4 z; z.x = z.y = z.z = z.w = 0;
    CSH_UNROLL
    for (int j = 0; j < 8; j++) *reinterpret_cast<uint4 *>(blk + CSH_OCT_STRIDE * j) = z;
}

#define CSH_NZF_CAP 2040u
#define CSH_NZF_CTL (4u * CSH_NZF_CAP)
#define CSH_NZF_PHASES 4
__device__ __forceinline__ static uint32_t nzf_ones(uint32_t w, uint32_t ones) {
#ifdef CSH_EMUL
    (void)ones;
    return ((w & 0xFFFFu) ? 1u : 0u) | ((w >> 16) ? 0x10000u : 0u);
#else
    uint32_t r;
    asm("v_pk_min_u16 %0, %1, %2" : "=v"(r) : "v"(w), "v"(ones));
    return r;
#endif
}
__device__ __forceinline__ static uint32_t nzf_count(const uint4 lv[8]) {
    uint32_t ones = 0x00010001u;
    CSH_PIN(ones);
    uint32_t s = 0;
    CSH_UNROLL
    for (int j = 0; j < 8; j++) { s += nzf_ones(lv[j].x, ones); s += nzf_ones(lv[j].y, ones); s += nzf_ones(lv[j].z, ones); s += nzf_ones(lv[j].w, ones); }
    s -= nzf_ones(lv[0].x, ones) & 1u;
    return (s & 0xFFFFu) + (s >> 16);
}
template <int K>
__device__ __forceinline__ static void nzf_put(uint32_t w, uint32_t kb, uint32_t *dst, uint32_t &o) {
    const int h = (K & 1) ? (int(w) >> 16) : (int(w << 16) >> 16);
    const uint32_t a = uint32_t(h < 0 ? -h : h);
    dst[o] = (kb | uint32_t(K)) | (h < 0 ? 128u : 0u) | (a << 8);
    o += h != 0 ? 1u : 0u;
}
template <int J>
__device__ __forceinline__ static void nzf_octet(const uint4 &v, uint32_t kb, uint32_t *dst, uint32_t &o) {
    uint32_t x = v.x, y = v.y, z = v.z, w = v.w;
    if ((x | y | z | w) == 0u) return;
    CSH_PIN(x); CSH_PIN(y); CSH_PIN(z); CSH_PIN(w);
    if (J) nzf_put<8 * J>(x, kb, dst, o);
    nzf_put<8 * J + 1>(x, kb, dst, o); nzf_put<8 * J + 2>(y, kb, dst, o); nzf_put<8 * J + 3>(y, kb, dst, o); nzf_put<8 * J + 4>(z, kb, dst, o);
    nzf_put<8 * J + 5>(z, kb, dst, o); nzf_put<8 * J + 6>(w, kb, dst, o); nzf_put<8 * J + 7>(w, kb, dst, o);
}
template <int... J>
__device__ __forceinline__ static void nzf_walk(const uint4 lv[8], uint32_t blk, bool real, uint32_t *dst, uint32_t o, std::integer_sequence<int, J...>) {
    if (!real) return;
    const uint32_t kb = blk << 23;
    ((nzf_octet<J>(lv[J], kb, dst, o), CSH_SCHED_FENCE()), ...);
    dst[o] = CSH_NZ_END | kb;
}
__device__ __forceinline__ static bool nzf_begin(const NzFuse &f, const PlaneWork &w, NzSet &S) {
    if (!f.nz_pool || w.nzset == 0xFFFFFFFFu) return false;
    S = f.nzsets[w.nzset];
    return blockIdx.x * 256u < S.nunits;
}
__device__ __forceinline__ static void nzf_counted(const NzSet &S, const uint4 lv[8], uint32_t ns[2], uint32_t *cnt_lds) {
    const uint32_t u = blockIdx.x * 256u + threadIdx.x;
    ns[0] = u < S.nunits ? nzf_count(lv) + 1u : 0u;
#ifdef CSH_EMUL
    cnt_lds[threadIdx.x] = ns[0];
#else
    (void)cnt_lds;
#endif
}
__device__ __forceinline__ static void nzf_phase(int phase, const NzFuse &f, const NzSet &S, const uint4 lv[8], uint32_t ns[2], uint32_t *lds, const uint32_t *cnt_lds) {
    const uint32_t tid = threadIdx.x, wave = tid >> 6, lane = tid & 63u, u = blockIdx.x * 256u + tid;
    const bool real = u < S.nunits;
    if (phase == 1) {
        uint32_t ex = 0, tot = 0;
#ifdef CSH_EMUL
        for (uint32_t i = 0; i < 64; i++) { const uint32_t n = cnt_lds[wave * 64u + i]; if (i < lane) ex += n; tot += n; }
#else
        (void)cnt_lds;
        LV<uint32_t> c; c.v = ns[0];
        ex = lscan(c, tot).v;
#endif
        ns[1] = ex;
        if (lane == 0) lds[CSH_NZF_CTL + wave] = tot;
        if (tot <= CSH_NZF_CAP) nzf_walk(lv, tid, real, lds + wave * CSH_NZF_CAP, ex, Oct());
        return;
    }
    if (phase == 2) {
        if (tid == 0) {
            const NzList L0 = f.nzlists[S.list[0]];
            const uint32_t n0 = lds[CSH_NZF_CTL] + lds[CSH_NZF_CTL + 1] + lds[CSH_NZF_CTL + 2] + lds[CSH_NZF_CTL + 3], n0a = (n0 + 3u) & ~3u, rec0 = L0.chunk0 + blockIdx.x;
            const uint32_t rel = atomicAdd(&f.nz_cursor[S.list[0]], n0a);
            const bool ok0 = uint64_t(rel) + n0a <= L0.cap;
            f.nz_chunk_off[rec0] = rel; f.nz_chunk_cnt[rec0] = ok0 ? n0 : 0u;
            if (!ok0) f.overflow[1] = 1;
            lds[CSH_NZF_CTL + 4] = ok0 ? rel : 0xFFFFFFFFu;
        }
        return;
    }
    const uint32_t rel = lds[CSH_NZF_CTL + 4];
    if (rel == 0xFFFFFFFFu) return;
    const uint32_t t0 = lds[CSH_NZF_CTL], t1 = lds[CSH_NZF_CTL + 1], t2 = lds[CSH_NZF_CTL + 2], t3 = lds[CSH_NZF_CTL + 3];
    const uint32_t wbase = uint32_t(CSH_UNIFORM((wave > 0 ? t0 : 0u) + (wave > 1 ? t1 : 0u) + (wave > 2 ? t2 : 0u)));
    const uint32_t tot = uint32_t(CSH_UNIFORM(wave == 0 ? t0 : wave == 1 ? t1 : wave == 2 ? t2 : t3)), n0 = t0 + t1 + t2 + t3;
    uint32_t *chunk = f.nz_pool + f.nzlists[S.list[0]].base + rel;
    if (tot <= CSH_NZF_CAP) {
        const uint32_t *src = lds + wave * CSH_NZF_CAP;
        for (uint32_t i = lane; i < tot; i += 64u) chunk[wbase + i] = src[i];
    } else {
// ... 4 lines not shown
        if (f.blk_off) f.blk_off[S.cnt_base + u] = uint16_t(wbase + ns[1]);
    }
    if (wave == 3u && n0 + lane < ((n0 + 3u) & ~3u)) chunk[n0 + lane] = 0u;
}
#ifdef CSH_EMUL
#define CSH_NZF_STATE CSH_SHARED uint32_t s_nzc[256]; CSH_PERSIST(uint4, lv, 8); CSH_PERSIST(uint32_t, ns, 2)
#define CSH_NZF_LOOP CSH_PHASE_LOOP(CSH_NZF_PHASES)
#define CSH_NZF_EARLY(x) x
#define CSH_NZF_LATE(x) ((void)0)
#define CSH_NZF_FINISH() ((void)0)
#else
#define CSH_NZF_STATE uint32_t *const s_nzc = nullptr; uint4 lv[8]; uint32_t ns[2] = {0u, 0u}
#define CSH_NZF_LOOP for (int phase = 0, once_ = 1; once_; once_ = 0)
#define CSH_NZF_EARLY(x) ((void)0)
#define CSH_NZF_LATE(x) x
#define CSH_NZF_FINISH()                                                                                                                  \
    do {                                                                                                                                   \
        if (!fuse) return;                                                                                                                 \
        CSH_UNROLL                                                                                                                         \
        for (int ph_ = 1; ph_ < CSH_NZF_PHASES; ph_++) { __syncthreads(); nzf_phase(ph_, nzf, S, lv, ns, reinterpret_cast<uint32_t *>(&s_dr[0][0]), s_nzc); } \
    } while (0)
#endif

template <bool DERING>
__global__ void __launch_bounds__(256) k_xform_direct(const ImgDesc *__restrict__ imgs, const PlaneWork *__restrict__ work, const DevQuant *__restrict__ quant,
                                                       const int16_t *__restrict__ coef_in, int16_t *__restrict__ coef_out, int16_t *__restrict__ dct_raw, uint32_t raw_tile0, NzFuse nzf) {
    CSH_SHARED int16_t s_dr[64][256];
    CSH_NZF_STATE;
    const PlaneWork w = work[blockIdx.y];
    if (w.mode != 0) return;
    const ImgDesc &im = imgs[w.image];
    const CompGeom gi = im.in[w.comp], go = im.out[w.comp];
    int tile = blockIdx.x * (blockDim.x >> 6) + (threadIdx.x >> 6);
    int lane = threadIdx.x & 63;
    int b = tile * 64 + lane;
    NzSet S;
    bool fuse = false;
    CSH_NZF_EARLY(fuse = nzf_begin(nzf, w, S));
    CSH_NZF_LOOP {
    if (phase) {
        if (!fuse) break;
        nzf_phase(phase, nzf, S, lv, ns, reinterpret_cast<uint32_t *>(&s_dr[0][0]), s_nzc);
        continue;
    }
    bool has_raw = false;
    do {
        if (b >= go.bw * go.bh) break;
        int by = b / go.bw, bx = b - by * go.bw;
        if (by >= go.real_bh || bx >= go.real_bw) { store_zero_block(coef_out + coef_index(go.tile_base, b, 0)); break; }
        int x[64];
        load_idct<true>(coef_in + coef_index(gi.tile_base, by * gi.bw + bx, 0), quant[CSH_UNIFORM(im.qt_in[w.comp])], x);
        int vc = gi.comp_w - bx * 8, vr = gi.comp_h - by * 8;
        if (vc < 8 || vr < 8) replicate_edges(x, vc, vr);
        fdct_quant_store<DERING, true>(x, quant[CSH_UNIFORM(im.qt_out[w.comp])], BlkOut{coef_out, go.tile_base, b, dct_raw, go.tile_base - raw_tile0}, lv, s_dr);
        has_raw = dct_raw != nullptr;
    } while (0);
    if (dct_raw) raw_copy_out(dct_raw + raw_index(go.tile_base - raw_tile0, tile * 64), has_raw, s_dr, int(threadIdx.x));
    CSH_NZF_LATE(fuse = nzf_begin(nzf, w, S));
    if (fuse) nzf_counted(S, lv, ns, s_nzc);
    }
    CSH_NZF_FINISH();
}

__global__ void __launch_bounds__(256) k_idct_plane(const ImgDesc *__restrict__ imgs, const PlaneWork *__restrict__ work, const DevQuant *__restrict__ quant,
                                                     const int16_t *__restrict__ coef_in, uint8_t *__restrict__ planes) {
    const PlaneWork w = work[blockIdx.y];
    if (w.mode == 0) return;
    const ImgDesc &im = imgs[w.image];
    const CompGeom gi = im.in[w.comp];
    int tile = blockIdx.x * (blockDim.x >> 6) + (threadIdx.x >> 6);
    int lane = threadIdx.x & 63;
    int b = tile * 64 + lane;
    if (b >= gi.bw * gi.bh) return;
    int by = b / gi.bw, bx = b - by * gi.bw;
    if (by >= gi.real_bh || bx >= gi.real_bw) return;
    int x[64];
    load_idct(coef_in + coef_index(gi.tile_base, b, 0), quant[CSH_UNIFORM(im.qt_in[w.comp])], x);
    int vc = gi.comp_w - bx * 8, vr = gi.comp_h - by * 8;
    if (vc < 8 || vr < 8) replicate_edges(x, vc, vr);
    int pitch = gi.real_bw * 8;
    uint8_t *p = planes + im.plane_off[w.comp] + size_t(by * 8) * pitch + bx * 8;
    CSH_UNROLL
    for (int r = 0; r < 8; r++) {
        uint32_t lo = uint32_t(x[8 * r]) | (uint32_t(x[8 * r + 1]) << 8) | (uint32_t(x[8 * r + 2]) << 16) | (uint32_t(x[8 * r + 3]) << 24);
        uint32_t hi = uint32_t(x[8 * r + 4]) | (uint32_t(x[8 * r + 5]) << 8) | (uint32_t(x[8 * r + 6]) << 16) | (uint32_t(x[8 * r + 7]) << 24);
        uint2 v; v.x = lo; v.y = hi;
        *reinterpret_cast<uint2 *>(p + size_t(r) * pitch) = v;
    }
}

struct PlaneView { const uint8_t *p; int pitch, cw, ch; };

__device__ __forceinline__ static int pv(const PlaneView &v, int y, int x) {
    y = y < 0 ? 0 : (y > v.ch - 1 ? v.ch - 1 : y);
    x = x < 0 ? 0 : (x > v.cw - 1 ? v.cw - 1 : x);
    return v.p[size_t(y) * v.pitch + x];
}
__device__ static int up_h2v2(const PlaneView &v, int r, int xx) {
    int cy = r >> 1, cx = xx >> 1;
    if (v.cw <= 2) return pv(v, cy, cx);
    int fy = (r & 1) ? cy + 1 : cy - 1;
    int nb = (xx & 1) ? cx + 1 : cx - 1;
    int cs = 3 * pv(v, cy, cx) + pv(v, fy, cx);
    int cn = 3 * pv(v, cy, nb) + pv(v, fy, nb);
    return (3 * cs + cn + ((xx & 1) ? 7 : 8)) >> 4;
}

// ... 174 lines not shown
    PlaneView v;
    v.p = planes + im.splane_off[w.comp]; v.pitch = gi.real_bw * 8; v.cw = gi.comp_w; v.ch = gi.comp_h;
    const int W = im.enc_w, H = im.enc_h, och = go.comp_h;
    const UpDesc u = w.up;
    uint32_t out;
    if (u.cls == CSH_UP_H2V2 && w.dn == CSH_DN_H4V1 && x0 >= 4 && 2 * x0 + 8 <= v.pitch && 4 * x0 + 15 <= W - 1) {
        const int ye = y < och - 1 ? y : och - 1;
        out = resample_quad_420_411(v, ye > H - 1 ? H - 1 : ye, x0);
    } else {
        switch (w.dn) {
        case CSH_DN_FULL: out = resample_any_quad<CSH_DN_FULL>(v, u, W, H, och, y, x0); break;
        case CSH_DN_H2V2: out = resample_any_quad<CSH_DN_H2V2>(v, u, W, H, och, y, x0); break;
        case CSH_DN_H2V1: out = resample_any_quad<CSH_DN_H2V1>(v, u, W, H, och, y, x0); break;
        default: out = resample_any_quad<CSH_DN_H4V1>(v, u, W, H, och, y, x0); break;
        }
    }
    *reinterpret_cast<uint32_t *>(oplanes + im.oplane_off[w.comp] + size_t(y) * pitch_o + x0) = out;
}

template <bool DERING>
__global__ void __launch_bounds__(256) k_plane_fdct(const ImgDesc *__restrict__ imgs, const PlaneWork *__restrict__ work, const DevQuant *__restrict__ quant, const uint8_t *__restrict__ oplanes,
                                                     int16_t *__restrict__ coef_out, int16_t *__restrict__ dct_raw, uint32_t raw_tile0, NzFuse nzf) {
    CSH_SHARED int16_t s_dr[64][256];
    CSH_NZF_STATE;
    const PlaneWork w = work[blockIdx.y];
    if (w.mode == 0 || w.mode == 10) return;
    const ImgDesc &im = imgs[w.image];
    const CompGeom go = im.out[w.comp];
    int tile = blockIdx.x * (blockDim.x >> 6) + (threadIdx.x >> 6);
    int lane = threadIdx.x & 63;
    int b = tile * 64 + lane;
    NzSet S;
    bool fuse = false;
    CSH_NZF_EARLY(fuse = nzf_begin(nzf, w, S));
    CSH_NZF_LOOP {
    if (phase) {
        if (!fuse) break;
        nzf_phase(phase, nzf, S, lv, ns, reinterpret_cast<uint32_t *>(&s_dr[0][0]), s_nzc);
        continue;
    }
    bool has_raw = false;
    do {
    if (b >= go.bw * go.bh) break;
    int by = b / go.bw, bx = b - by * go.bw;
    if (by >= go.real_bh || bx >= go.real_bw) { store_zero_block(coef_out + coef_index(go.tile_base, b, 0)); break; }
    const int pitch = go.real_bw * 8;
    const uint8_t *p = oplanes + im.oplane_off[w.comp] + size_t(by * 8) * pitch + bx * 8;
    uint32_t pr[8][4];
    CSH_UNROLL
    for (int r = 0; r < 8; r++) {
        const uint2 v = *reinterpret_cast<const uint2 *>(p + size_t(r) * pitch);
        pr[r][0] = bytes_to_halves<0, 1>(v.x); pr[r][2] = bytes_to_halves<2, 3>(v.x); pr[r][1] = bytes_to_halves<3, 2>(v.y); pr[r][3] = bytes_to_halves<1, 0>(v.y);
    }
    fdct_quant_store_pk<DERING, false>(pr, quant[CSH_UNIFORM(im.qt_out[w.comp])], BlkOut{coef_out, go.tile_base, b, dct_raw, go.tile_base - raw_tile0}, lv, s_dr);
    has_raw = dct_raw != nullptr;
    } while (0);
    if (dct_raw) raw_copy_out(dct_raw + raw_index(go.tile_base - raw_tile0, tile * 64), has_raw, s_dr, int(threadIdx.x));
    CSH_NZF_LATE(fuse = nzf_begin(nzf, w, S));
    if (fuse) nzf_counted(S, lv, ns, s_nzc);
    }
    CSH_NZF_FINISH();
}

struct Row16 { uint32_t a, b, c, d; };
__device__ __forceinline__ static Row16 load_row16(const uint8_t *p) {
    Row16 r;
#ifdef CSH_EMUL
    __builtin_memcpy(&r, p, 16);
#else
    typedef uint32_t u32x4_a4 __attribute__((ext_vector_type(4), aligned(4)));
    const u32x4_a4 v = *reinterpret_cast<const u32x4_a4 *>(p);
    r.a = v.x; r.b = v.y; r.c = v.z; r.d = v.w;
#endif
    return r;
}
template <bool DERING>
__global__ void __launch_bounds__(256) k_resample_fdct_420(const ImgDesc *__restrict__ imgs, const PlaneWork *__restrict__ work, const DevQuant *__restrict__ quant, const uint8_t *__restrict__ planes,
                                                            int16_t *__restrict__ coef_out, int16_t *__restrict__ dct_raw, uint32_t raw_tile0, NzFuse nzf) {
    CSH_SHARED int16_t s_dr[64][256];
    CSH_NZF_STATE;
    const PlaneWork w = work[blockIdx.y];
    if (w.mode != 10) return;
    const ImgDesc &im = imgs[w.image];
    const CompGeom gi = im.src[w.comp], go = im.out[w.comp];
    int tile = blockIdx.x * (blockDim.x >> 6) + (threadIdx.x >> 6);
    int lane = threadIdx.x & 63;
    int b = tile * 64 + lane;
    NzSet S;
    bool fuse = false;
    CSH_NZF_EARLY(fuse = nzf_begin(nzf, w, S));
    CSH_NZF_LOOP {
    if (phase) {
        if (!fuse) break;
        nzf_phase(phase, nzf, S, lv, ns, reinterpret_cast<uint32_t *>(&s_dr[0][0]), s_nzc);
        continue;
    }
    bool has_raw = false;
    do {
    if (b >= go.bw * go.bh) break;
    int by = b / go.bw, bx = b - by * go.bw;
    if (by >= go.real_bh || bx >= go.real_bw) { store_zero_block(coef_out + coef_index(go.tile_base, b, 0)); break; }
    const int pitch = gi.real_bw * 8, rows_alloc = gi.real_bh * 8;
    const uint8_t *pl = planes + im.splane_off[w.comp];
    const int x0 = bx * 8, y0 = by * 8, W = im.enc_w, H = im.enc_h, och = go.comp_h;
    const bool first = bx == 0, last = x0 + 12 > pitch, hodd = (H & 1) != 0;
    const int kt = ((W - 1) >> 1) - x0;
    uint32_t mA[2], mB[2], mC[2], mD[2];
// ... 17 lines not shown
    }
    const bool patch = kt < 8 && ((mA[0] | mB[0] | mC[0] | mD[0] | mA[1] | mB[1] | mC[1] | mD[1]) != 0u);
#ifdef CSH_EMUL
    const bool any_patch = patch;
#else
    const bool any_patch = __ballot(patch) != 0ull;
#endif
    uint32_t pr[8][4];
    Quad420 win[3][2];
    auto row_fields = [&](int j, Quad420 out[2]) {
        const uint32_t bq = rows[j].b, cq = rows[j].c;
        const uint32_t aq = first ? bq << 24 : rows[j].a;
        const uint32_t dq = last ? cq >> 24 : rows[j].d;
        out[0] = quad420_fields(aq, bq, cq);
        out[1] = quad420_fields(bq, cq, dq);
    };
    row_fields(0, win[0]);
    row_fields(1, win[1]);
    CSH_UNROLL
    for (int r = 0; r < 8; r++) {
        Quad420 *p = win[r % 3], *c = win[(r + 1) % 3], *n = win[(r + 2) % 3];
        row_fields(r + 2, n);
        Sums420 s[2] = {quad420_sums(p[0], c[0], n[0]), quad420_sums(p[1], c[1], n[1])};
        if (any_patch && patch) {
            const int odd_col = kt & 1;
            const Sums420 &sq = (kt >> 2) ? s[1] : s[0];
            const uint32_t sqA = (kt >> 2) ? s[1].A : s[0].A, sqB = (kt >> 2) ? s[1].B : s[0].B, sqC = (kt >> 2) ? s[1].C : s[0].C, sqD = (kt >> 2) ? s[1].D : s[0].D;
            (void)sq;
            uint32_t sl = wodd ? (odd_col ? sqC : sqA) : (odd_col ? sqD : sqB);
            sl = (kt & 2) ? sl >> 16 : sl & 0xFFFFu;
            sl |= sl << 16;
            CSH_UNROLL
            for (int qq = 0; qq < 2; qq++) {
                s[qq].A = (s[qq].A & ~mA[qq]) | (sl & mA[qq]);
                s[qq].B = (s[qq].B & ~mB[qq]) | (sl & mB[qq]);
                s[qq].C = (s[qq].C & ~mC[qq]) | (sl & mC[qq]);
                s[qq].D = (s[qq].D & ~mD[qq]) | (sl & mD[qq]);
            }
        }
        uint32_t e0, o0, e1, o1;
        quad420_finish(s[0], e0, o0);
        quad420_finish(s[1], e1, o1);
        pr[r][0] = pack_halves(e0, o0); pr[r][2] = pack_hi_halves(e0, o0); pr[r][1] = pack_hi_halves(o1, e1); pr[r][3] = pack_halves(o1, e1);
    }
    const int ylast = och - 1 - y0;
    if (ylast < 7) {
        CSH_UNROLL
        for (int r = 1; r < 8; r++)
            if (r > ylast) {
                CSH_UNROLL
                for (int cc = 0; cc < 4; cc++) pr[r][cc] = pr[r - 1][cc];
            }
    }
    fdct_quant_store_pk<DERING, false>(pr, quant[CSH_UNIFORM(im.qt_out[w.comp])], BlkOut{coef_out, go.tile_base, b, dct_raw, go.tile_base - raw_tile0}, lv, s_dr);
    has_raw = dct_raw != nullptr;
    } while (0);
    if (dct_raw) raw_copy_out(dct_raw + raw_index(go.tile_base - raw_tile0, tile * 64), has_raw, s_dr, int(threadIdx.x));
    CSH_NZF_LATE(fuse = nzf_begin(nzf, w, S));
    if (fuse) nzf_counted(S, lv, ns, s_nzc);
    }
    CSH_NZF_FINISH();
}

__global__ void __launch_bounds__(256) k_requant(const ImgDesc *__restrict__ imgs, const PlaneWork *__restrict__ work, const DevQuant *__restrict__ quant, const int16_t *__restrict__ dct_raw, uint32_t raw_tile0,
                                                  int16_t *__restrict__ coef_out) {
    const PlaneWork w = work[blockIdx.y];
    const ImgDesc &im = imgs[w.image];
    const CompGeom go = im.out[w.comp];
    int tile = blockIdx.x * (blockDim.x >> 6) + (threadIdx.x >> 6);
    int lane = threadIdx.x & 63;
    int b = tile * 64 + lane;
    if (b >= go.bw * go.bh) return;
    int by = b / go.bw, bx = b - by * go.bw;
    if (by >= go.real_bh || bx >= go.real_bw) return;
    requant_block(dct_raw + raw_index(go.tile_base - raw_tile0, b), quant[CSH_UNIFORM(im.qt_out[w.comp])], coef_out + coef_index(go.tile_base, b, 0), Oct());
}

__global__ void k_fix_dummy(const ImgDesc *imgs, int nimg, int16_t *coef_out) {
    int i = blockIdx.y;
    if (i >= nimg) return;
    const ImgDesc &im = imgs[i];
    int t = blockIdx.x * blockDim.x + threadIdx.x;
    for (int c = 0; c < im.ncomp; c++) {
        const CompGeom &g = im.out[c];
        int ndummy_cols = g.bw - g.real_bw, ndummy_rows = g.bh - g.real_bh;
        int n_right = ndummy_cols * g.real_bh, n_bottom = ndummy_rows * g.bw;
        if (t < n_right) {
            int by = t / ndummy_cols, bx = g.real_bw + t % ndummy_cols;
            coef_out[coef_index(g.tile_base, by * g.bw + bx, 0)] = coef_out[coef_index(g.tile_base, by * g.bw + g.real_bw - 1, 0)];
        } else if (t - n_right < n_bottom) {
            int u = t - n_right;
            int by = g.real_bh + u / g.bw, bx = u % g.bw;
            int sx = (bx / g.h) * g.h + g.h - 1;
            if (sx > g.real_bw - 1) sx = g.real_bw - 1;
            coef_out[coef_index(g.tile_base, by * g.bw + bx, 0)] = coef_out[coef_index(g.tile_base, (g.real_bh - 1) * g.bw + sx, 0)];
        }
    }
}

static dim3 tile_grid(int max_tiles, int nwork) { return dim3((max_tiles + 3) / 4, nwork); }

void launch_xform_direct(hipStream_t st, const ImgDesc *imgs, const PlaneWork *work, int nwork, int max_tiles, const DevQuant *quant,
                         const int16_t *coef_in, int16_t *coef_out, int16_t *dct_raw, uint32_t raw_tile0, bool dering, const NzFuse &nzf) {
    if (!nwork) return;
    if (dering) CSH_LAUNCH_PHASED(k_xform_direct<true>, CSH_NZF_PHASES, tile_grid(max_tiles, nwork), dim3(256), st, imgs, work, quant, coef_in, coef_out, dct_raw, raw_tile0, nzf);
    else CSH_LAUNCH_PHASED(k_xform_direct<false>, CSH_NZF_PHASES, tile_grid(max_tiles, nwork), dim3(256), st, imgs, work, quant, coef_in, coef_out, dct_raw, raw_tile0, nzf);
}
// ... 32 lines not shown
```

caesium-clt_amd/csrc/k_trellis.hip:

```cpp
#include <algorithm>
#include <atomic>
#include <cassert>
#include <utility>

#include "kernels.h"

namespace csh {

#define CSH_TR_CAP 16
#define CSH_TR_WGU uint32_t(CSH_TR_WG)
#define CSH_TR_SPILL (63 - CSH_TR_CAP)
#define CSH_TR_MAXWG 2048
size_t trellis_spill_words(uint32_t nslots) { return size_t(nslots) * CSH_TR_SPILL * 3u * CSH_TR_WGU; }

#ifdef CSH_EMUL
#define CSH_ANY(p) (p)
#define CSH_WAVE_OR(v) (v)
#define CSH_SPILL_LD(ptr) (*(ptr))
#define CSH_SPILL_ST(ptr, v) (*(ptr) = (v))
#else
#define CSH_ANY(p) (__ballot(p) != 0ull)
__device__ __forceinline__ static unsigned tr_wave_or(unsigned v) {
    const unsigned n = 32u - unsigned(__clz(v));
    unsigned r = 0;
// ... 166 lines not shown
                    }
                    CSH_UNROLL
                    for (int i = 0; i < 4; i++) {
                        CSH_UNROLL
                        for (int kc = 0; kc < KC; kc++) {
                            const bool better = cost[i][kc] < bestc;
                            bestc = better ? cost[i][kc] : bestc;
                            bestsel = better ? ((uint32_t(j0 + i + 1) << 4) | uint32_t(kc)) : bestsel;
                        }
                    }
                }
            };
            if (ncmax <= 1) batch(std::integral_constant<int, 1>());
            else if (ncmax == 2) batch(std::integral_constant<int, 2>());
            else if (ncmax == 3) batch(std::integral_constant<int, 3>());
            else batch(std::integral_constant<int, 4>());
        } else
            for (int jj = 0; jj < t_lds; jj++) from(jj, int((L.P[jj][tid] >> 15) & 63u), L.A[jj][tid], L.Z[jj][tid]);
        for (int jj = CSH_TR_CAP; jj < int(t); jj++) {
            const uint32_t *q = sp + (uint32_t(jj - CSH_TR_CAP) * 3u) * CSH_TR_WGU;
            from(jj, int((CSH_SPILL_LD(q + 2 * CSH_TR_WG) >> 15) & 63u), tr_bits_f(CSH_SPILL_LD(q)), tr_bits_f(CSH_SPILL_LD(q + CSH_TR_WG)));
        }
        if (on) {
            const int bk = int(bestsel & 15u);
            const uint32_t level = uint32_t(bk < ncand - 1 ? (2 << bk) - 1 : qval);
            const float Zi = (float(__mul24(x, x)) * lambda) * ltk + Zp;
            const uint32_t P2 = (bestsel >> 4) | ((level == uint32_t(qval) && qval < TRELLIS_MAX_LEVEL) ? 0x4000u : 0u) | (uint32_t(kpos) << 15) | (level << 21) | (P & 0x80000000u);
            if (t < CSH_TR_CAP) { L.A[t][tid] = bestc; L.Z[t][tid] = Zi; L.P[t][tid] = P2; }
            else { uint32_t *q = sp + ((t - CSH_TR_CAP) * 3u) * CSH_TR_WGU; CSH_SPILL_ST(q, tr_f_bits(bestc)); CSH_SPILL_ST(q + CSH_TR_WG, tr_f_bits(Zi)); CSH_SPILL_ST(q + 2 * CSH_TR_WG, P2); }
        }
    }

    float best = Z63 + lenEOBf;
    int last = -1;
    for (uint32_t e = 0; CSH_ANY(e < ne); e++) {
        float Ae, Ze; uint32_t Pe;
        if (e < CSH_TR_CAP) { Ae = L.A[e][tid]; Ze = L.Z[e][tid]; Pe = L.P[e][tid]; }
        else { const uint32_t *q = sp + ((e - CSH_TR_CAP) * 3u) * CSH_TR_WGU; Ae = tr_bits_f(CSH_SPILL_LD(q)); Ze = tr_bits_f(CSH_SPILL_LD(q + CSH_TR_WG)); Pe = CSH_SPILL_LD(q + 2 * CSH_TR_WG); }
        float cost = (Ae + Z63) - Ze;
        if (int((Pe >> 15) & 63u) < 63) cost = cost + lenEOBf;
        if (e < ne && cost < best) { best = cost; last = int(e); }
    }

    if (c.debug & 4u) return;
    uint64_t kept = 0;
    for (int e = last; CSH_ANY(e >= 0);) {
        if (e >= 0) {
            uint32_t Pe;
            if (e < CSH_TR_CAP) Pe = L.P[e][tid]; else Pe = CSH_SPILL_LD(sp + (uint32_t(e - CSH_TR_CAP) * 3u + 2u) * CSH_TR_WGU);
            kept |= 1ull << e;
            e = int(Pe & 63u) - 1;
        }
    }
    int16_t *dst = c.coef + coef_index(g.tile_base, b, 0);
    uint32_t *lst = nullptr;
    if (c.nz_pool && w.nzset != 0xFFFFFFFFu) {
        const NzSet &S = c.nzsets[w.nzset];
        const NzList &L0 = c.nzlists[S.list[0]];
        const uint32_t rec = L0.chunk0 + (u >> 8);
        if (c.nz_chunk_cnt[rec]) lst = c.nz_pool + L0.base + c.nz_chunk_off[rec] + c.blk_off[w.unit_base + u];
    }
    uint32_t room = ne;
    if (lst && c.blk_cnt) {
        room = c.blk_cnt[w.unit_base + u];
#ifdef CSH_EMUL
        if (room != ne) { fprintf(stderr, "k_trellis_ac: block %u of unit %u has %u list entries but %u levels\n", u, w.unit_base, room, ne); abort(); }
#endif
    }
    for (uint32_t e0 = 0; CSH_ANY(e0 < ne); e0 += 4) {
        uint32_t ent[4] = {0u, 0u, 0u, 0u};
        CSH_UNROLL
        for (uint32_t i = 0; i < 4; i++) {
            const uint32_t e = e0 + i;
            if (e < ne) {
                uint32_t Pe;
                if (e < CSH_TR_CAP) Pe = L.P[e][tid]; else Pe = CSH_SPILL_LD(sp + ((e - CSH_TR_CAP) * 3u + 2u) * CSH_TR_WGU);
                const int pos = int((Pe >> 15) & 63u), level = ((kept >> e) & 1ull) ? int((Pe >> 21) & 1023u) : 0;
                if (!(((kept >> e) & 1ull) && (Pe & 0x4000u))) dst[coef_off(pos)] = int16_t((Pe >> 31) ? -level : level);
                ent[i] = uint32_t(pos) | ((Pe >> 31) ? 128u : 0u) | (uint32_t(level) << 8) | ((u & 255u) << 23);
            }
        }
        if (lst && e0 < ne && e0 < room) {
            if (e0 + 4 <= ne && e0 + 4 <= room) {
#ifdef CSH_EMUL
                memcpy(lst + e0, ent, 16);
#else
                typedef uint32_t tr_u32x4_a4 __attribute__((ext_vector_type(4), aligned(4)));
                tr_u32x4_a4 v; v.x = ent[0]; v.y = ent[1]; v.z = ent[2]; v.w = ent[3];
                *reinterpret_cast<tr_u32x4_a4 *>(lst + e0) = v;
#endif
            } else {
                CSH_UNROLL
                for (uint32_t i = 0; i < 4; i++) if (e0 + i < ne && e0 + i < room) lst[e0 + i] = ent[i];
            }
        }
    }
}

__global__ void __launch_bounds__(256) k_trellis_sort(TrellisCtx c) {
    CSH_SHARED uint32_t s_cnt[64];
    const TrellisWork w = c.work[blockIdx.x];
    const uint8_t *cnt = c.blk_cnt + w.unit_base;
    uint32_t *perm = c.perm + w.unit_base;
    CSH_PHASE_LOOP(4) {
        if (phase == 0) { if (threadIdx.x < 64) s_cnt[threadIdx.x] = 0; continue; }
        if (phase == 1) { for (uint32_t u = threadIdx.x; u < w.nunits; u += 256) atomicAdd(&s_cnt[cnt[u] & 63u], 1u); continue; }
        if (phase == 2) {
            if (threadIdx.x == 0) { uint32_t at = 0; for (int k = 63; k >= 0; k--) { const uint32_t n = s_cnt[k]; s_cnt[k] = at; at += n; } }
            continue;
        }
        for (uint32_t u = threadIdx.x; u < w.nunits; u += 256) perm[atomicAdd(&s_cnt[cnt[u] & 63u], 1u)] = u;
    }
}
void launch_trellis_sort(hipStream_t st, const TrellisCtx &c) { if (c.nwork && c.perm && c.blk_cnt) CSH_LAUNCH_PHASED(k_trellis_sort, 4, dim3(unsigned(c.nwork)), dim3(256), st, c); }

__global__ void __launch_bounds__(CSH_TR_WG) k_trellis_ac(TrellisCtx c) {
    CSH_SHARED float s_A[CSH_TR_CAP][CSH_TR_WG];
    CSH_SHARED float s_Z[CSH_TR_CAP][CSH_TR_WG];
    CSH_SHARED uint32_t s_P[CSH_TR_CAP][CSH_TR_WG];
    CSH_SHARED float s_lenf[16 * 11 + 16];
    CSH_SHARED float s_runf[4];
    CSH_SHARED int s_eob;
    CSH_SHARED int32_t s_q8[64];
    CSH_SHARED uint32_t s_qmul[64];
    CSH_SHARED uint32_t s_qsh[64];
    CSH_SHARED float s_lt[64];
    CSH_SHARED float s_rcp[64];
    TrLds L; L.A = s_A; L.Z = s_Z; L.P = s_P; L.lenf = s_lenf; L.runf = s_runf; L.q8 = s_q8; L.qmul = s_qmul; L.qsh = s_qsh; L.lt = s_lt; L.rcp = s_rcp;
#ifdef CSH_EMUL
    CSH_PHASE_LOOP(2) {
        const TrellisRun rn = c.runs[blockIdx.x];
// ... 172 lines not shown
```

caesium-clt_amd/csrc/kernels.h:

```cpp
#pragma once
#include "gpu_rt.h"
#include "types.h"

namespace csh {

__host__ __device__ static inline int coef_off(int k) { return (k >> 3) * CSH_OCT_STRIDE + (k & 7); }
__host__ __device__ static inline size_t coef_index(uint32_t tile_base, int b, int k) {
    return (size_t(tile_base) + size_t(b >> 6)) * CSH_TILE_I16 + size_t((b & 63) * CSH_BLK_STRIDE) + size_t(coef_off(k));
}

#define CSH_RAW_OCT 8
__host__ __device__ static inline size_t raw_index(uint32_t tile_base, int b) { return size_t(tile_base) * CSH_TILE_I16 + size_t(b) * 64; }

__device__ __forceinline__ static int csh_plane_at(const uint8_t *p, int pitch, int cw, int ch, int y, int x) {
    y = y < 0 ? 0 : (y > ch - 1 ? ch - 1 : y);
    x = x < 0 ? 0 : (x > cw - 1 ? cw - 1 : x);
    return p[size_t(y) * pitch + x];
}
__device__ __forceinline__ static int csh_upsample_at(const uint8_t *p, int pitch, int cw, int ch, UpDesc u, int r, int xx) {
    switch (u.cls) {
    case CSH_UP_COPY: return csh_plane_at(p, pitch, cw, ch, r, xx);
    case CSH_UP_H2V1: {
        const int cx = xx >> 1, nb = (xx & 1) ? cx + 1 : cx - 1;
        return (3 * csh_plane_at(p, pitch, cw, ch, r, cx) + csh_plane_at(p, pitch, cw, ch, r, nb) + ((xx & 1) ? 2 : 1)) >> 2;
// ... 83 lines not shown
    uint64_t *sym_bits;
    uint64_t *eob_bits;
    uint8_t *tail;
    uint16_t *eobrun;
    uint32_t *long_runs, *long_cnt;
    uint64_t *corr;
    uint32_t *tokens;
    const TokRegion *regions;
    uint32_t *tok_cursor;
    uint64_t *tok_off;
    uint32_t *chunk_ntok;
    uint16_t *slot_hist;
    uint32_t *slot_raw;
    uint32_t *slot_eobh;
    uint32_t *chunk_bits;
    const uint64_t *chunk_off;
    DevEncTable *tables;
    uint32_t *raw;
    uint64_t raw_words;
    uint32_t *status;
    uint32_t *overflow;
    uint32_t debug;
    uint32_t stats_only;
    const uint8_t *work_active;
    const NzList *nzlists;
    const NzSet *nzsets;
    const NzChunk *nzchunks;
    uint32_t nnzchunks;
    uint32_t *nz_pool;
    uint32_t *nz_cursor;
    uint32_t *nz_chunk_off;
    uint32_t *nz_chunk_cnt;
    uint8_t *nz_blk_cnt;
    uint16_t *nz_blk_off;
    const uint32_t *list_slots;
    uint32_t nlist_slots;
    const uint32_t *tok_slots;
    uint32_t ntok_slots;
    const uint32_t *ref_slots;
    uint32_t nref_slots;
    uint32_t nz_build, nz_filter;
};
enum : uint32_t { TK_SYM = 0u, TK_RAW = 1u, TK_ACF = 2u, TK_REF = 3u, TK_EOB = 4u };
void launch_tokens(hipStream_t st, const EncCtx &c);
void launch_ac_runs(hipStream_t st, const EncCtx &c);
void launch_gen_tables(hipStream_t st, DevEncTable *tables, int ntables);
void launch_chunk_sizes(hipStream_t st, const EncCtx &c);
void launch_zero_edges(hipStream_t st, const EncCtx &c);
void launch_pack(hipStream_t st, const EncCtx &c);
void launch_nzlist(hipStream_t st, const EncCtx &c);
void launch_list_stats(hipStream_t st, const EncCtx &c);
void launch_list_refine(hipStream_t st, const EncCtx &c);
void launch_list_pack(hipStream_t st, const EncCtx &c);
void launch_reset_works(hipStream_t st, ScanWork *work, int nwork);

#ifndef CSH_TR_WG
#define CSH_TR_WG 256
#endif
#ifndef CSH_TR_RUN
#define CSH_TR_RUN 8
#endif
struct TrellisCtx {
    const ImgDesc *imgs;
    const DevQuant *quant;
    const TrellisWork *work;
    int nwork;
    const TrellisRun *runs;
    uint32_t nruns;
    uint32_t *queue;
    uint32_t nslots;
    const DevEncTable *tables;
    const int16_t *raw;
    uint32_t raw_tile0;
    int16_t *coef;
    uint64_t *dcrec;
    uint64_t *dcbt;
    uint32_t *spill;
    uint32_t max_rows;
    const uint8_t *blk_cnt;
    uint32_t *perm;
    const uint32_t *rows;
    uint32_t nrows;
    uint32_t debug;
    uint32_t *nz_pool;
    const NzList *nzlists;
    const NzSet *nzsets;
    const uint32_t *nz_chunk_off, *nz_chunk_cnt;
    const uint16_t *blk_off;
};
void launch_trellis_sort(hipStream_t st, const TrellisCtx &c);
void launch_trellis_ac(hipStream_t st, const TrellisCtx &c);
void launch_trellis_dc(hipStream_t st, const TrellisCtx &c);
uint32_t trellis_ac_slots();
size_t trellis_spill_words(uint32_t nslots);

void launch_exclusive_scan(hipStream_t st, const uint32_t *in, uint64_t *out, uint64_t n, void *tmp, size_t tmp_bytes);
size_t exclusive_scan_tmp_bytes(uint64_t n);

struct AsmCtx {
    const ImgDesc *imgs;
    const EncScan *script;
    ScanWork *work;
    int nwork, nimg, scans_per_image;
    int work0, nwork_run;
    const uint32_t *img_list;
    const uint32_t *img_nlist;
    uint32_t *scan_cost;
    const DevEncTable *tables;
    const uint64_t *chunk_off;
    uint32_t *scan_pad_bytes;
    uint64_t *scan_raw_off;
    const uint32_t *raw;
    uint64_t raw_chunks;
    uint32_t *chunk_ff;
    const uint8_t *hdr_pool;
    const uint32_t *hdr_off;
    uint32_t *img_size_pad;
    uint32_t *img_size;
    uint64_t *img_off;
    uint8_t *out;
    uint64_t out_cap;
    uint32_t *status;
    uint32_t *overflow;
};
void launch_scan_cost(hipStream_t st, const AsmCtx &a);
void launch_scan_sizes(hipStream_t st, const AsmCtx &a);
void launch_scan_place(hipStream_t st, const AsmCtx &a);
void launch_ff_count(hipStream_t st, const AsmCtx &a);
void launch_layout(hipStream_t st, const AsmCtx &a);
void launch_emit(hipStream_t st, const AsmCtx &a);

}
```

caesium-clt_amd/csrc/pipeline.cpp:

```cpp
#include <algorithm>
#include <atomic>
#include <cmath>
#include <cstdarg>
#include <memory>
#include <thread>

#include "batch.hpp"
#include "../../include/vp8_tables.h"
#include "resize_host.h"

static thread_local char g_err[512];
void csh_set_error(const char *fmt, ...) {
    va_list ap;
    va_start(ap, fmt);
    vsnprintf(g_err, sizeof g_err, fmt, ap);
    va_end(ap);
}
extern "C" const char *csh_last_error(void) { return g_err; }

#ifdef CSH_EMUL
thread_local dim3 threadIdx, blockIdx, blockDim, gridDim;
int csh_emul_reverse = 0;
thread_local int csh_emul_phase = 0;
extern "C" void csh_emul_set_reverse(int r) { csh_emul_reverse = r; }
// ... 171 lines not shown
    CSH_CHECK(hipStreamSynchronize(b->stream));
    return 0;
}
extern "C" int csh_batch_rerun_encode(csh_batch *b, csh_timing *t) {
    if (!b->have_dct) { csh_set_error("rerun_encode needs a completed csh_batch_run after csh_batch_retain_dct(1)"); return -1; }
    return batch_run(b, t, true);
}

static int batch_run(csh_batch *b, csh_timing *t, bool requant_only) {
    if (t) memset(t, 0, sizeof *t);
    if (!b->nimg) { b->out.ran = true; return 0; }
    if (hipSetDevice(b->device) != hipSuccess) { csh_set_error("hipSetDevice failed"); return CS_ERR_NO_DEVICE; }
    for (int attempt = 0; attempt < 4; attempt++) {
        if (run_once(b, t, requant_only)) return CS_ERR_NO_DEVICE;
        uint32_t ovf[4] = {0, 0, 0, 0};
        if (csh_copy_wait(ovf, b->out.d_overflow.p, sizeof ovf, hipMemcpyDeviceToHost, b->stream) != hipSuccess) { csh_set_error("D2H failed"); return CS_ERR_NO_DEVICE; }
        b->out.h_status.resize(b->nimg);
        if (csh_copy_wait(b->out.h_status.data(), b->out.d_status.p, b->nimg * sizeof(uint32_t), hipMemcpyDeviceToHost, b->stream) != hipSuccess) return CS_ERR_NO_DEVICE;
        bool pool = ovf[0] != 0;
        if (ovf[1]) {
            pool = true; b->enc.tok_scale *= 4;
            layout_token_pool(b);
            if (b->enc.d_regions.upload(b->enc.regions, b->stream) || b->enc.d_nzlists.upload(b->enc.nzlists, b->stream) || hipStreamSynchronize(b->stream) != hipSuccess) return CS_ERR_NO_DEVICE;
        }
        for (uint32_t s : b->out.h_status) if (s == CS_ERR_POOL_OVERFLOW) pool = true;
        if (!pool) break;
        if (attempt == 3) { csh_set_error("device pools overflowed after 3 retries"); return CS_ERR_POOL_OVERFLOW; }
        b->out.raw_bytes_cap *= 4; b->out.out_cap = b->out.raw_bytes_cap;
        b->wp.webp_mb_bytes *= 4;
    }
    b->out.h_img_size.resize(b->nimg);
    b->out.h_img_off.resize(b->nimg + 1);
    if (csh_copy_wait(b->out.h_img_size.data(), b->out.d_img_size.p, b->nimg * sizeof(uint32_t), hipMemcpyDeviceToHost, b->stream) != hipSuccess ||
        csh_copy_wait(b->out.h_img_off.data(), b->out.d_img_off.p, (b->nimg + 1) * sizeof(uint64_t), hipMemcpyDeviceToHost, b->stream) != hipSuccess) {
        csh_set_error("D2H of sizes failed"); return CS_ERR_NO_DEVICE;
    }
    if (t) {
        std::vector<uint32_t> ns(b->nimg);
        if (csh_copy_wait(ns.data(), b->dec.d_need_seq.p, b->nimg * sizeof(uint32_t), hipMemcpyDeviceToHost, b->stream) != hipSuccess) return CS_ERR_NO_DEVICE;
        if (getenv("CSH_TRACE") && b->dec.d_relax_cnt.n) {
            std::vector<uint32_t> rc(b->dec.d_relax_cnt.n);
            if (csh_copy_wait(rc.data(), b->dec.d_relax_cnt.p, rc.size() * sizeof(uint32_t), hipMemcpyDeviceToHost, b->stream) == hipSuccess) {
                fprintf(stderr, "[csh] relax list sizes (of %u sub-sequences):", b->dec.total_sub);
                for (size_t i = 0; i < rc.size() && (i < 16 || rc[i]); i++) fprintf(stderr, " %u", rc[i]);
                fprintf(stderr, "\n");
            }
        }
        for (const ProgChain &pc : b->dec.chains) if (pc.refine && ns[size_t(pc.image)] == 4) t->n_refine_chains++;
        for (uint32_t v : ns) { if (v == 4) { t->n_prog_decoded++; continue; } if (v) t->n_seq_decoded++; if (v == 2 || v == 3) t->n_par_fallback++; if (v == 3) t->n_par_short++; }
        t->n_images = uint32_t(b->nimg);
        t->n_search_extra = b->enc.search ? b->enc.n_gated_runs : 0u;
        t->n_fused_lists = b->enc.last_run_fused;
        t->n_list_refine = b->enc.last_run_refine;
        for (const Item &it : b->items) if (it.image < 0) t->n_failed++;
        for (int i = 0; i < b->nimg; i++) { t->out_bytes += b->out.h_img_size[i]; t->pixels += uint64_t(b->imgs[i].width) * b->imgs[i].height; }
        t->in_bytes = b->dec.bits_pool.size();
        uint64_t in_tiles = 0;
        for (const ImgDesc &im : b->imgs) for (int c = 0; c < im.ncomp; c++) in_tiles += im.in[c].ntiles;
        t->coef_bytes = in_tiles * CSH_TILE_I16 * 2;
    }
    b->out.ran = true;
    if (!requant_only) b->have_dct = (b->retain_dct || b->tr.trellis) && !b->lossless;
    return 0;
}

static void set_result(CCSResult *r, int code, const std::string &msg) {
    r->success = code == 0;
    r->code = uint32_t(code);
    r->error_message = nullptr;
    if (code) { char *m = (char *)malloc(msg.size() + 1); memcpy(m, msg.c_str(), msg.size() + 1); r->error_message = m; }
}

extern "C" int csh_batch_pixels(csh_batch *b, size_t image, const uint8_t **device_pixels, uint32_t *width, uint32_t *height, uint32_t *channels, const char **message) {
    *device_pixels = nullptr; *width = *height = *channels = 0;
    if (message) *message = "";
    if (!b || !b->out.ran || !b->rgb_out || image >= b->items.size()) { csh_set_error("csh_batch_pixels: not a pixel batch that has run"); if (message) *message = "not a pixel batch that has run"; return CS_ERR_NO_DEVICE; }
    const Item &it = b->items[image];
    if (it.code) { if (message) *message = it.msg.c_str(); return it.code; }
    if (b->out.h_status[it.image]) { if (message) *message = "device reported a malformed stream"; return int(b->out.h_status[it.image]); }
    if (size_t(it.image) < b->pix.rwork.size() && b->pix.rwork[size_t(it.image)].image == it.image) {
        const ResizeWork &rw = b->pix.rwork[size_t(it.image)];
        *device_pixels = b->pix.d_rgb.p + rw.rgb_dst_off; *width = uint32_t(rw.nw); *height = uint32_t(rw.nh); *channels = uint32_t(b->imgs[it.image].ncomp);
        return 0;
    }
    if (message) *message = "image has no pixel output";
    return CS_ERR_NO_DEVICE;
}

extern "C" int csh_batch_fetch(csh_batch *b, CByteArray *outputs, CCSResult *results) {
    if (!b->out.ran) { csh_set_error("csh_batch_fetch before csh_batch_run"); return -1; }
    if (b->rgb_out) { csh_set_error("csh_batch_fetch: a pixel batch has no files (csh_batch_pixels)"); return -1; }
    struct PinnedOut { uint8_t *p = nullptr; size_t cap = 0; ~PinnedOut() { if (p) pinned_cache().put(p, cap); } uint8_t *data() const { return p; } } host;
    if (b->nimg && b->out.h_img_off[b->nimg]) {
        host.p = static_cast<uint8_t *>(pinned_cache().get(b->out.h_img_off[b->nimg], host.cap));
        if (!host.p) { csh_set_error("out of pinned host memory"); return -1; }
        if (csh_copy_wait(host.p, b->out.d_out.p, b->out.h_img_off[b->nimg], hipMemcpyDeviceToHost, b->stream) != hipSuccess) { csh_set_error("D2H of output failed"); return -1; }
    }
    std::atomic<int> failed{0};
    std::atomic<size_t> next{0};
    auto worker = [&]() {
        for (size_t n; (n = next++) < b->items.size();) {
            Item &it = b->items[n];
            outputs[n].data = nullptr; outputs[n].length = 0;
            int code = it.code;
            std::string msg = it.msg;
            if (!code && it.image >= 0 && b->out.h_status[it.image]) { code = int(b->out.h_status[it.image]); msg = "device reported a malformed stream"; }
            if (!code) {
                size_t len = b->out.h_img_size[it.image];
                outputs[n].data = (uint8_t *)malloc(len ? len : 1);
                memcpy(outputs[n].data, host.data() + b->out.h_img_off[it.image], len);
                outputs[n].length = len;
            } else failed++;
            if (results) set_result(&results[n], code, msg);
        }
    };
    size_t nthreads = std::min<size_t>(std::min<size_t>(8, std::max(1u, std::thread::hardware_concurrency())), b->items.size() / 64 + 1);
    std::vector<std::thread> pool;
    for (size_t t = 1; t < nthreads; t++) pool.emplace_back(worker);
    worker();
    for (auto &t : pool) t.join();
    return failed.load();
}

extern "C" int csh_batch_geometry(csh_batch *b, size_t image, int comp, int which, int *bw, int *bh, int *real_bw, int *real_bh) {
    if (image >= b->items.size() || b->items[image].image < 0) { csh_set_error("image not on the device"); return -1; }
    const ImgDesc &im = b->imgs[b->items[image].image];
    if (comp < 0 || comp >= im.ncomp) { csh_set_error("bad component"); return -1; }
    const CompGeom &g = which ? im.out[comp] : im.in[comp];
    *bw = g.bw; *bh = g.bh; *real_bw = g.real_bw; *real_bh = g.real_bh;
    return 0;
}

extern "C" int csh_batch_read_coefs(csh_batch *b, size_t image, int comp, int which, int16_t *dst) {
    int bw, bh, rbw, rbh;
    if (csh_batch_geometry(b, image, comp, which, &bw, &bh, &rbw, &rbh)) return -1;
    const ImgDesc &im = b->imgs[b->items[image].image];
    const CompGeom &g = which ? im.out[comp] : im.in[comp];
    std::vector<int16_t> tiles(size_t(g.ntiles) * CSH_TILE_I16);
    if (csh_copy_wait(tiles.data(), b->d_coef.p + size_t(g.tile_base) * CSH_TILE_I16, tiles.size() * 2, hipMemcpyDeviceToHost, b->stream) != hipSuccess) { csh_set_error("D2H failed"); return -1; }
    for (int blk = 0; blk < bw * bh; blk++)
        for (int k = 0; k < 64; k++) dst[size_t(blk) * 64 + k] = tiles[size_t(blk >> 6) * CSH_TILE_I16 + (blk & 63) * CSH_BLK_STRIDE + coef_off(k)];
    return 0;
}
```

caesium-clt_amd/csrc/types.h:

```cpp
#pragma once
#include <cstdint>

#define CSH_TILE_BLOCKS 64
#define CSH_TILE_I16 4096
#ifndef CSH_BLOCK_MAJOR
#define CSH_BLOCK_MAJOR 0
#endif
#if CSH_BLOCK_MAJOR
#define CSH_OCT_STRIDE 8
#define CSH_BLK_STRIDE 64
#else
#define CSH_OCT_STRIDE 512
#define CSH_BLK_STRIDE 8
#endif
#define CSH_MAX_COMPS 3
#define CSH_MASK_PLANES 6
#define CSH_MASK_TILE (CSH_MASK_PLANES * 64)
#define CSH_MAX_SCANS 20
#define CSH_LIST_MAX 16

namespace csh {

struct CompGeom {
    int h, v;
// ... 45 lines not shown
    CompGeom in[CSH_MAX_COMPS];
    CompGeom out[CSH_MAX_COMPS];
    int qt_in[CSH_MAX_COMPS];
    int qt_out[CSH_MAX_COMPS];
    uint64_t plane_off[CSH_MAX_COMPS];
    uint64_t oplane_off[CSH_MAX_COMPS];
    CompGeom src[CSH_MAX_COMPS];
    uint64_t splane_off[CSH_MAX_COMPS];
    int enc_w, enc_h;
    int first_scan, nscans_in;
    int comp_id[CSH_MAX_COMPS];
    int first_work, nscans_out;
    uint32_t status;
};

#define CSH_SUBSEQ_BYTES 128
struct ParScan {
    uint32_t bits_off, bits_len;
    uint32_t clean_len;
    int huff_set, image, ncomp;
    int nb_mcu;
    int comp_of[10], by_of[10], bx_of[10], dct[10], act[10];
    uint32_t total_blocks;
    uint32_t sub_base;
    uint32_t par_index;
    uint32_t dc_base[10], dc_per_mcu[10], dc_idx[10];
    uint64_t sel;
    uint32_t first_mcu;
    int kind;
    int Ss, Se, Al;
};
enum { CSH_PS_SEQ = 0, CSH_PS_UNSTUFF = 1, CSH_PS_DC_FIRST = 2, CSH_PS_AC_FIRST = 3, CSH_PS_DC_REFINE = 4 };

struct DevQuant {
    uint16_t q[64];
    int32_t div[64];
    float rcp[64];
    float lt[64];
    uint32_t mul[64];
    uint32_t sh[64];
};

enum { CSH_UP_COPY = 0, CSH_UP_H2V2 = 1, CSH_UP_H2V1 = 2, CSH_UP_H1V2 = 3, CSH_UP_REP = 4 };
enum { CSH_DN_FULL = 0, CSH_DN_H2V2 = 1, CSH_DN_H2V1 = 2, CSH_DN_H4V1 = 3 };
struct UpDesc { uint8_t cls, hx, vx, pad; };

#define CSH_MODE_ANY 11
struct PlaneWork {
    int image, comp;
    int mode;
    UpDesc up;
    int dn;
    uint32_t nzset;
};

#define CSH_RZ_ANY (-2)
struct ResizeWork {
    int image, in_kind;
    UpDesc up[CSH_MAX_COMPS];
    int nw, nh;
    uint64_t rgb_src_off, rgb_dst_off;
    uint64_t tmp_off;
    uint32_t vtap_base, htap_base;
};
struct ResizeTap { int left, n; uint32_t woff; };

struct EncScan {
    int ncomp, comp[CSH_MAX_COMPS];
    int Ss, Se, Ah, Al;
    int dc_tbl[CSH_MAX_COMPS];
    int ac_tbl[CSH_MAX_COMPS];
    int sequential;
    int ntables;
    int dht_id[4];
    int sos_tdta[CSH_MAX_COMPS];
};

struct ScanWork {
    int image, scan;
    uint32_t nunits;
    uint32_t unit_base;
    uint32_t first_chunk;
    uint32_t word_base;
    uint32_t table_base;
    uint32_t ff_bytes;
    uint64_t raw_off;
    uint32_t raw_bytes;
    uint32_t out_off;
    uint32_t hdr_bytes;
    uint32_t no_room;
    uint32_t list;
    uint32_t corr_base;
    uint32_t hist_row0;
    uint32_t ls_base;
    uint32_t rs_base;
    uint32_t region;
};

struct EChunk { uint32_t a; uint16_t comp, kind; uint32_t j; uint32_t plan; uint32_t region; };
struct TokRegion { uint64_t base; uint32_t cap, pad; };
#define CSH_TK_MAXSLOT 12
struct AcSlot { uint32_t unit_base, word_base, first_chunk, table_base, nunits_work; uint8_t Ss, Se, Ah, Al; uint32_t corr_base, pad; };
struct TokPlan {
    uint32_t nslot, nunits;
    int32_t real_bw, bw;
    uint32_t tile_base;
    uint32_t work0;
    uint32_t pad[2];
    AcSlot s[CSH_TK_MAXSLOT];
};
#define CSH_NZ_END 64u
#define CSH_NZ_LEVELS 4
struct NzList {
    uint64_t base;
    uint32_t cap;
    uint32_t chunk0;
};
struct NzSet {
    uint32_t list[CSH_NZ_LEVELS];
    uint32_t nunits;
    int32_t real_bw, bw;
    uint32_t tile_base;
    uint32_t cnt_base;
    uint32_t pad[3];
};
#define CSH_NZ_COMPACT0 0x80000000u
struct NzChunk { uint32_t set, j, levels, work0; };

struct SlotRec {
    uint32_t work, j, nch;
    uint32_t first_chunk;
    uint32_t unit0, nun;
    uint32_t table_base;
    uint16_t ntables, flags;
    uint32_t hist_row;
    uint32_t word_base, unit_base, nunits_work;
    uint8_t Ss, Se, Ah, Al; uint32_t corr0;
    uint32_t nzlist, nzrec;
    uint32_t region;
};

struct TrellisWork {
    int image, comp;
    uint32_t table_ac;
    int32_t table_dc;
    uint32_t nunits;
    uint32_t unit_base;
    uint32_t nzset;
    uint32_t pad[1];
};
struct TrellisRun { uint32_t work, j, n; };

struct DevEncTable {
    uint32_t freq[257];
    uint8_t bits[17];
    uint8_t vals[256];
    uint16_t code[256];
    uint8_t size[256];
    int nsym;
    uint32_t lut[256];
};

}
```

include/caesium_hip.h:

```cpp
#ifndef CAESIUM_HIP_H
#define CAESIUM_HIP_H
#include <stdbool.h>
#include <stddef.h>
#include <stdint.h>
#ifdef __cplusplus
extern "C" {
#endif

enum { CS_TYPE_JPEG = 0, CS_TYPE_PNG = 1, CS_TYPE_GIF = 2, CS_TYPE_WEBP = 3, CS_TYPE_TIFF = 4, CS_TYPE_UNKN = 5 };

enum {
    CS_OK = 0,
    CS_ERR_NO_DEVICE = 10001,
    CS_ERR_UNKNOWN_TYPE = 10200,
    CS_ERR_UNSUPPORTED = 10201,
    CS_ERR_BAD_JPEG = 20100,
    CS_ERR_JPEG_FEATURE = 20101,
    CS_ERR_POOL_OVERFLOW = 20200,
    CS_ERR_BAD_PNG = 30100,
    CS_ERR_BAD_WEBP = 40100,
    CS_ERR_SAME_FORMAT = 10407,
    CS_ERR_TOO_BIG = 10500
};

// ... 15 lines not shown
    uint32_t tiff_deflate_level;
    uint32_t width;
    uint32_t height;
} CCSParameters;

typedef struct {
    bool success;
    uint32_t code;
    const char *error_message;
} CCSResult;

typedef struct {
    uint8_t *data;
    size_t length;
} CByteArray;

void cs_default_parameters(CCSParameters *p);

CCSResult cs_compress_in_memory(const uint8_t *in, size_t n, const CCSParameters *p, CByteArray *out);
CCSResult cs_compress_to_size_in_memory(const uint8_t *in, size_t n, CCSParameters *p, size_t max_output_size,
                                        bool return_smallest, CByteArray *out);
CCSResult cs_convert_in_memory(const uint8_t *in, size_t n, const CCSParameters *p, uint32_t format, CByteArray *out);
int cs_batch_convert(const CByteArray *inputs, size_t count, const CCSParameters *p, uint32_t format, int device, CByteArray *outputs, CCSResult *results);

int cs_batch_compress(const CByteArray *inputs, size_t count, const CCSParameters *p, int device,
                      CByteArray *outputs, CCSResult *results);
int cs_batch_compress_to_size(const CByteArray *inputs, size_t count, CCSParameters *p, size_t max_output_size, bool return_smallest,
                              int device, CByteArray *outputs, CCSResult *results);

size_t cs_batch_extent(const CByteArray *inputs, size_t count);

void cs_free_bytes(CByteArray *b);
void cs_free_result(CCSResult *r);

typedef struct csh_batch csh_batch;

enum { CSH_NPHASES = 8, CSH_NKERNELS = 36 };
typedef struct {
    float total_ms;
    float phase_ms[CSH_NPHASES];
    float kernel_ms[CSH_NKERNELS];
    uint64_t in_bytes, out_bytes;
    uint64_t pixels;
    uint64_t coef_bytes;
    uint32_t n_images, n_failed;
    uint32_t n_seq_decoded;
    uint32_t n_par_fallback;
    uint32_t n_par_short;
    uint32_t n_prog_decoded;
    uint32_t n_refine_chains;
    uint32_t n_search_extra;
    uint32_t n_fused_lists;
    uint32_t n_list_refine;
} csh_timing;

int csh_device_count(void);
const char *csh_last_error(void);
void csh_warmup(int device);
void csh_release_cached_memory(void);
const char *csh_kernel_name(int slot);
const char *csh_kernel_name_webp(int slot);
int csh_batch_create(const CByteArray *inputs, size_t count, const CCSParameters *p, int device, csh_batch **out);
int csh_batch_create_webp(const CByteArray *inputs, size_t count, const CCSParameters *p, int device, csh_batch **out);
int csh_batch_create_pixels(const CByteArray *inputs, size_t count, const CCSParameters *p, int device, csh_batch **out);
int csh_batch_pixels(csh_batch *b, size_t image, const uint8_t **device_pixels, uint32_t *width, uint32_t *height, uint32_t *channels, const char **message);
struct csp_pixels_s;
int csh_batch_create_from_pixels(const struct csp_pixels_s *sources, size_t count, const CCSParameters *p, int device, csh_batch **out);
int csh_batch_run(csh_batch *b, csh_timing *t);
int csh_batch_fetch(csh_batch *b, CByteArray *outputs, CCSResult *results);
void csh_batch_destroy(csh_batch *b);

int csh_batch_retain_dct(csh_batch *b, int on);
int csh_batch_set_quality(csh_batch *b, const uint32_t *quality);
int csh_batch_rerun_encode(csh_batch *b, csh_timing *t);

int csh_batch_geometry(csh_batch *b, size_t image, int comp, int which, int *bw, int *bh, int *real_bw, int *real_bh);
int csh_batch_read_coefs(csh_batch *b, size_t image, int comp, int which, int16_t *dst);

typedef struct csp_batch csp_batch;
enum { CSP_NKERNELS = 16 };
typedef struct {
    float total_ms;
    float kernel_ms[CSP_NKERNELS];
    uint64_t in_bytes, out_bytes;
    uint64_t pixels, raw_bytes;
    uint32_t n_images, n_failed, n_trials;
} csp_timing;
const char *csp_kernel_name(int slot);
int csp_batch_create(const CByteArray *inputs, size_t count, const CCSParameters *p, int device, csp_batch **out);
int csp_batch_create_webp(const CByteArray *inputs, size_t count, const CCSParameters *p, int device, csp_batch **out);
typedef struct csp_pixels_s { const uint8_t *device_pixels; uint32_t width, height, channels; } csp_pixels;
int csp_batch_create_pixels(const csp_pixels *sources, size_t count, const CCSParameters *p, int device, csp_batch **out);
int csp_png_to_jpeg(const CByteArray *inputs, size_t count, const CCSParameters *p, int device, CByteArray *outputs, CCSResult *results);
int csp_png_to_lossless_webp(const CByteArray *inputs, size_t count, const CCSParameters *p, int device, CByteArray *outputs, CCSResult *results);
int csp_batch_run(csp_batch *b, csp_timing *t);
int csp_batch_fetch(csp_batch *b, CByteArray *outputs, CCSResult *results);
void csp_batch_destroy(csp_batch *b);
int csp_batch_geometry(csp_batch *b, size_t image, uint32_t *width, uint32_t *height, uint32_t *rowbytes);
int csp_batch_read_rows(csp_batch *b, size_t image, uint8_t *dst);
int csp_batch_read_stream(csp_batch *b, size_t image, int strategy, uint8_t *dst);
int csp_batch_read_scores(csp_batch *b, size_t image, uint64_t *dst, int *have);
int csp_batch_trials(csp_batch *b, size_t image, int *strategies, uint64_t *zlib_bytes, int *ntrials, int *winner);
int csp_batch_chunk_bits(csp_batch *b, size_t image, int trial, uint64_t *dst, size_t cap, size_t *nchunks);

int csl_encode_pixels(const struct csp_pixels_s *sources, size_t count, int device, CByteArray *outputs, CCSResult *results);
int csl_attach_alpha(CByteArray *lossy, const CByteArray *alpha_vp8l, uint32_t width, uint32_t height);
// ... 20 lines not shown
```

Before: 43220.

## Keep AC coefficients only in nonzero lists for progressive fused planes

For progressive encodes where the fused nonzero-list path and list refinement are active, the pixel/DCT kernels and the trellis now write only the DC octet of each block to the coefficient tiles. AC coefficients live only in the nonzero lists, which removes most of the coefficient-tile store traffic. When coefficients are read back for inspection, a new kernel rebuilds the tiles from the lists. The gain depends on every downstream stage really reading AC data from the lists; planes that still have a token plan are excluded, and a debug memset option helps catch stale tile reads.

```diff
diff --git a/caesium-clt_amd/binding.py b/caesium-clt_amd/binding.py
--- a/caesium-clt_amd/binding.py
+++ b/caesium-clt_amd/binding.py
@@ -25,7 +25,7 @@
 
 class Timing(C.Structure):
     _fields_ = [("total_ms", C.c_float), ("phase_ms", C.c_float * NPHASES), ("kernel_ms", C.c_float * NKERNELS), ("in_bytes", C.c_uint64), ("out_bytes", C.c_uint64),
-                ("pixels", C.c_uint64), ("coef_bytes", C.c_uint64), ("n_images", C.c_uint32), ("n_failed", C.c_uint32), ("n_seq_decoded", C.c_uint32), ("n_par_fallback", C.c_uint32), ("n_par_short", C.c_uint32), ("n_prog_decoded", C.c_uint32), ("n_refine_chains", C.c_uint32), ("n_search_extra", C.c_uint32), ("n_fused_lists", C.c_uint32), ("n_list_refine", C.c_uint32)]
+                ("pixels", C.c_uint64), ("coef_bytes", C.c_uint64), ("n_images", C.c_uint32), ("n_failed", C.c_uint32), ("n_seq_decoded", C.c_uint32), ("n_par_fallback", C.c_uint32), ("n_par_short", C.c_uint32), ("n_prog_decoded", C.c_uint32), ("n_refine_chains", C.c_uint32), ("n_search_extra", C.c_uint32), ("n_fused_lists", C.c_uint32), ("n_list_refine", C.c_uint32), ("n_ac_in_lists", C.c_uint32)]
 
 
 class PngTiming(C.Structure):
diff --git a/caesium-clt_amd/csrc/batch.hpp b/caesium-clt_amd/csrc/batch.hpp
--- a/caesium-clt_amd/csrc/batch.hpp
+++ b/caesium-clt_amd/csrc/batch.hpp
@@ -116,6 +116,9 @@
     std::vector<NzChunk> nzchunks_fused;
     uint32_t n_fused = 0;
     uint32_t last_run_fused = 0;
+    uint32_t n_ac_lists = 0;
+    uint32_t last_run_ac_lists = 0;
+    std::vector<uint8_t> nzset_ac_lists;
     std::vector<uint32_t> nz_est, nz_worst;
     uint32_t nz_nrec = 0;
     uint64_t nz_cap = 0;
@@ -272,6 +275,7 @@
     bool fused_420 = true;
     bool nz_fused = true;
     bool ref_list = true;
+    bool ac_tiles = false;
     static PlanSwitches read();
 };
 
diff --git a/caesium-clt_amd/csrc/batch_plan.cpp b/caesium-clt_amd/csrc/batch_plan.cpp
--- a/caesium-clt_amd/csrc/batch_plan.cpp
+++ b/caesium-clt_amd/csrc/batch_plan.cpp
@@ -216,6 +216,7 @@
     s.nz_once = !is("CSH_NZ_ONCE", "0");
     s.tr_sort = !is("CSH_TR_SORT", "0");
     s.nz_fused = !is("CSH_NZ_FUSED", "0");
+    s.ac_tiles = is("CSH_AC_TILES", "1");
     s.ref_list = is("CSH_REF_LIST", "1") || (s.ref_list && !is("CSH_REF_LIST", "0"));
     const char *pp = getenv("CSH_PROG_PAR");
     s.prog_par = pp && !strcmp(pp, "0") ? 0 : (pp && !strcmp(pp, "1") ? 1 : -1);
@@ -713,7 +714,7 @@
 
 void BatchPlanner::plane_work(ImgDesc &im, const JpegInfo &in, const JpegInfo &o, int img_index, bool resized) {
     for (int c = 0; c < in.ncomp; c++) {
-        PlaneWork w; w.image = img_index; w.comp = c; w.nzset = 0xFFFFFFFFu;
+        PlaneWork w; w.image = img_index; w.comp = c; w.nzset = 0xFFFFFFFFu; w.ac_lists = 0u;
         w.up = resized ? up_desc(1, 1, 0) : up_desc(in.hmax / in.comp[c].h, in.vmax / in.comp[c].v, in.comp[c].comp_w);
         w.dn = dn_kind(o.hmax / o.comp[c].h, o.vmax / o.comp[c].v);
         const int in_kind = (w.up.hx == 1 && w.up.vx == 1) ? 0 : (w.up.hx == 2 && w.up.vx == 2) ? 1 : (w.up.hx == 2 && w.up.vx == 1) ? 2 : -1;
@@ -988,14 +989,24 @@
         b->enc.nzchunks_fused = b->enc.nzchunks;
         const bool allowed = sw.nz_fused && !b->lossless && !b->webp && !b->rgb_out && !(b->tr.trellis && progressive && !b->tr.nz_once);
         std::vector<uint8_t> fused(b->enc.nzsets.size(), 0);
+        const bool lists_only = progressive && !sw.ac_tiles && sw.ref_list && sw.nz_once && sw.tr_sort && (!b->tr.trellis || (b->tr.t_sort && b->tr.nz_once));
+        std::vector<uint8_t> planned(b->enc.nzsets.size(), 0);
+        for (size_t i = 0; i < b->enc.plans.size(); i++) {
+            const size_t at = size_t(b->enc.plan_image[i]) * CSH_MAX_COMPS + size_t(b->enc.plan_comp[i]);
+            if (at < b->enc.nzset_of.size() && b->enc.nzset_of[at] >= 0) planned[size_t(b->enc.nzset_of[at])] = 1;
+        }
+        b->enc.nzset_ac_lists.assign(b->enc.nzsets.size(), 0);
         for (PlaneWork &w : b->pix.pwork) {
+            w.ac_lists = 0u;
             const size_t at = size_t(w.image) * CSH_MAX_COMPS + size_t(w.comp);
             const int si = allowed && at < b->enc.nzset_of.size() ? b->enc.nzset_of[at] : -1;
             if (si < 0) continue;
             const NzSet &S = b->enc.nzsets[size_t(si)];
             if (S.real_bw != S.bw || S.list[0] == 0xFFFFFFFFu) continue;
             w.nzset = uint32_t(si); fused[size_t(si)] = 1; b->enc.n_fused++;
-        }
+            if (lists_only && !planned[size_t(si)]) { w.ac_lists = 1u; b->enc.nzset_ac_lists[size_t(si)] = 1; b->enc.n_ac_lists++; }
+        }
+        for (TrellisWork &tw : b->tr.twork) tw.ac_lists = (tw.nzset != 0xFFFFFFFFu && b->enc.nzset_ac_lists[tw.nzset]) ? 1u : 0u;
         for (NzChunk &ch : b->enc.nzchunks_fused) if (fused[ch.set]) ch.levels &= ~1u;
         auto flags = [&](Stage &sg) {
             for (int f = 0; f < 2; f++) {
diff --git a/caesium-clt_amd/csrc/batch_run.cpp b/caesium-clt_amd/csrc/batch_run.cpp
--- a/caesium-clt_amd/csrc/batch_run.cpp
+++ b/caesium-clt_amd/csrc/batch_run.cpp
@@ -189,6 +189,8 @@
             nzf.blk_cnt = (b->tr.trellis && b->tr.t_sort) ? b->tr.d_tblk_cnt.p : nullptr;
             nzf.blk_off = (nzf.blk_cnt && b->tr.nz_once) ? b->tr.d_tblk_off.p : nullptr;
         }
+        if (nw && getenv("CSH_DEBUG") && (uint32_t(atoi(getenv("CSH_DEBUG"))) & 32768u))
+            CSH_CHECK(hipMemsetAsync(b->d_coef.p + size_t(b->ntiles_in) * CSH_TILE_I16, 0x5A, size_t(b->ntiles - b->ntiles_in) * CSH_TILE_I16 * sizeof(int16_t), st));
         launch_xform_direct(st, b->d_imgs.p, b->pix.d_pwork.p, nw, b->max_tiles, b->d_quants.p, b->d_coef.p, b->d_coef.p, rawp, b->ntiles_in, b->tr.dering, nzf);
         MARK(KS_XFORM_DIRECT);
         launch_resample_plane(st, b->d_imgs.p, b->pix.d_pwork.p, nw, b->pix.max_quads, b->pix.d_planes.p, b->pix.d_oplanes.p);
@@ -235,6 +237,7 @@
             tc.nz_pool = b->enc.d_nz_pool.p; tc.nzlists = b->enc.d_nzlists.p; tc.nzsets = b->enc.d_nzsets.p; tc.nz_chunk_off = b->enc.d_nz_chunk_off.p; tc.nz_chunk_cnt = b->enc.d_nz_chunk_cnt.p;
             tc.blk_off = b->tr.d_tblk_off.p;
         }
+        tc.ac_lists = fused ? 1u : 0u;
         tc.debug = getenv("CSH_TR_DEBUG") ? uint32_t(atoi(getenv("CSH_TR_DEBUG"))) : 0u;
     }
 
@@ -406,7 +409,7 @@
 
 int run_once(csh_batch *b, csh_timing *t, bool requant_only) {
     Run r(b, t);
-    b->enc.last_run_fused = 0; b->enc.last_run_refine = 0;
+    b->enc.last_run_fused = 0; b->enc.last_run_refine = 0; b->enc.last_run_ac_lists = 0;
     if (r.pools() || r.marks.start()) return -1;
     const bool from_pixels = requant_only && b->tr.dering;
     if (requant_only && !from_pixels) {
@@ -420,6 +423,7 @@
     }
     if (r.encode_begin()) return -1;
     b->enc.last_run_fused = r.fused ? b->enc.n_fused : 0u;
+    b->enc.last_run_ac_lists = r.fused ? b->enc.n_ac_lists : 0u;
     if (b->tr.trellis ? r.trellis() : r.marks.skip_to(KS_NZLIST)) return -1;
     r.fill_asm_ctx();
     if (r.stage(b->enc.stage[0], true, false)) return -1;
diff --git a/caesium-clt_amd/csrc/k_aclist.hip b/caesium-clt_amd/csrc/k_aclist.hip
--- a/caesium-clt_amd/csrc/k_aclist.hip
+++ b/caesium-clt_amd/csrc/k_aclist.hip
@@ -210,6 +210,38 @@
             if (l == 0) c.nz_chunk_cnt[L0.chunk0 + ch.j] = n0new;
         }
     }
+}
+
+__global__ void __launch_bounds__(256) k_nz_to_tiles(const NzSet *nzsets, const NzList *nzlists, const uint32_t *nz_pool, const uint32_t *nz_chunk_off, const uint32_t *nz_chunk_cnt, uint32_t set,
+                                                      int16_t *coef) {
+    const NzSet S = nzsets[set];
+    const NzList L0 = nzlists[S.list[0]];
+    const uint32_t j = blockIdx.x, u0 = j * 256u;
+    CSH_PHASE_LOOP(2) {
+        if (phase == 0) {
+            const uint32_t u = u0 + threadIdx.x;
+            if (u >= S.nunits) continue;
+            const int by = int(u) / S.real_bw, bx = int(u) - by * S.real_bw;
+            int16_t *blk = coef + coef_index(S.tile_base, by * S.bw + bx, 0);
+            uint4 z; z.x = z.y = z.z = z.w = 0u;
+            z.x = uint32_t(uint16_t(blk[0]));
+            CSH_UNROLL
+            for (int o = 0; o < 8; o++) { *reinterpret_cast<uint4 *>(blk + CSH_OCT_STRIDE * o) = z; z.x = 0u; }
+            continue;
+        }
+        const uint32_t n = nz_chunk_cnt[L0.chunk0 + j];
+        const uint32_t *src = nz_pool + L0.base + nz_chunk_off[L0.chunk0 + j];
+        for (uint32_t i = threadIdx.x; i < n; i += 256u) {
+            const uint32_t e = src[i], k = e & 127u, u = u0 + ((e >> 23) & 255u);
+            if (k == 0u || k >= CSH_NZ_END || u >= S.nunits) continue;
+            const int by = int(u) / S.real_bw, bx = int(u) - by * S.real_bw, m = int((e >> 8) & 0x7FFFu);
+            coef[coef_index(S.tile_base, by * S.bw + bx, int(k))] = int16_t((e & 128u) ? -m : m);
+        }
+    }
+}
+void launch_nz_to_tiles(hipStream_t st, const NzSet *nzsets, const NzList *nzlists, const uint32_t *nz_pool, const uint32_t *nz_chunk_off, const uint32_t *nz_chunk_cnt, uint32_t set,
+                        uint32_t nchunks, int16_t *coef) {
+    if (nchunks) CSH_LAUNCH_PHASED(k_nz_to_tiles, 2, dim3(nchunks), dim3(256), st, nzsets, nzlists, nz_pool, nz_chunk_off, nz_chunk_cnt, set, coef);
 }
 
 struct NzEvent { uint32_t coded, term, run, size, bits, has, eob, blk; };
diff --git a/caesium-clt_amd/csrc/k_pixel.hip b/caesium-clt_amd/csrc/k_pixel.hip
--- a/caesium-clt_amd/csrc/k_pixel.hip
+++ b/caesium-clt_amd/csrc/k_pixel.hip
@@ -139,20 +139,20 @@
     return float_bits(__builtin_fmaf(float(x[kZ2N[K]]), q.rcp[K], 12582912.0f));
 }
 template <int J>
-__device__ __forceinline__ static void quant_store_octet(const int x[64], const DevQuant &q, int16_t *__restrict__ blk , uint4 &v) {
+__device__ __forceinline__ static void quant_store_octet(const int x[64], const DevQuant &q, int16_t *__restrict__ blk , uint4 &v, bool dc_only) {
     v.x = pack_halves(quant_one<8 * J + 0>(x, q), quant_one<8 * J + 1>(x, q));
     v.y = pack_halves(quant_one<8 * J + 2>(x, q), quant_one<8 * J + 3>(x, q));
     v.z = pack_halves(quant_one<8 * J + 4>(x, q), quant_one<8 * J + 5>(x, q));
     v.w = pack_halves(quant_one<8 * J + 6>(x, q), quant_one<8 * J + 7>(x, q));
-    nt_store16(blk + CSH_OCT_STRIDE * (J & 3), v);
+    if (J == 0 || !dc_only) nt_store16(blk + CSH_OCT_STRIDE * (J & 3), v);
 }
 template <int... J>
-__device__ __forceinline__ static void quant_store_all(const int x[64], const DevQuant &q, int16_t *__restrict__ blk, uint4 lv[8], std::integer_sequence<int, J...>) {
+__device__ __forceinline__ static void quant_store_all(const int x[64], const DevQuant &q, int16_t *__restrict__ blk, uint4 lv[8], bool dc_only, std::integer_sequence<int, J...>) {
     int16_t *hi = blk + 4 * CSH_OCT_STRIDE;
 #ifndef CSH_EMUL
     asm volatile("" : "+v"(hi));
 #endif
-    ((quant_store_octet<J>(x, q, J < 4 ? blk : hi, lv[J]), CSH_SCHED_FENCE()), ...);
+    ((quant_store_octet<J>(x, q, J < 4 ? blk : hi, lv[J], dc_only), CSH_SCHED_FENCE()), ...);
 }
 template <int J>
 __device__ __forceinline__ static void raw_store_octet(const int x[64], int16_t *__restrict__ raw) {
@@ -334,7 +334,7 @@
         pr[r][0] = pack_halves(at(0), at(1)); pr[r][1] = pack_halves(at(7), at(6)); pr[r][2] = pack_halves(at(2), at(3)); pr[r][3] = pack_halves(at(5), at(4));
     }
 }
-struct BlkOut { int16_t *coef_out; uint32_t tile_base; int b; int16_t *dct_raw; uint32_t raw_tile_base; };
+struct BlkOut { int16_t *coef_out; uint32_t tile_base; int b; int16_t *dct_raw; uint32_t raw_tile_base; bool dc_only;  };
 template <bool DERING, bool CENTRED>
 __device__ __forceinline__ static void fdct_quant_store_pk(uint32_t pr[8][4], const DevQuant &q, const BlkOut &o, uint4 lv[8], CSH_DERING_LDS) {
     CSH_SCHED_FENCE();
@@ -360,7 +360,7 @@
     if (o.dct_raw) {
         if (CSH_RAW_VIA_LDS) raw_put_all(x, dr_col, int(threadIdx.x), Oct()); else raw_store_all(x, o.dct_raw + raw_index(o.raw_tile_base, b), Oct());
     }
-    quant_store_all(x, q, o.coef_out + coef_index(o.tile_base, b, 0), lv, Oct());
+    quant_store_all(x, q, o.coef_out + coef_index(o.tile_base, b, 0), lv, o.dc_only, Oct());
 }
 __device__ __forceinline__ static void pack_rows(const int x[64], uint32_t pr[8][4]) {
     CSH_UNROLL
@@ -378,7 +378,7 @@
 template <bool DERING, bool CENTRED = false>
 __device__ __forceinline__ static void fdct_quant_store(int x[64], const DevQuant &q, int16_t *__restrict__ blk, int16_t *__restrict__ raw, CSH_DERING_LDS) {
     uint4 lv[8];
-    fdct_quant_store<DERING, CENTRED>(x, q, BlkOut{blk, 0u, 0, raw, 0u}, lv, dr_col);
+    fdct_quant_store<DERING, CENTRED>(x, q, BlkOut{blk, 0u, 0, raw, 0u, false}, lv, dr_col);
 }
 
 template <int J, int... I>
@@ -391,7 +391,7 @@
     int x[64];
     (raw_to_nat<J>(x, v[J], Oct()), ...);
     uint4 lv[8];
-    quant_store_all(x, q, blk, lv, Oct());
+    quant_store_all(x, q, blk, lv, false, Oct());
 }
 
 __device__ __forceinline__ static void store_zero_block(int16_t *__restrict__ blk) {
@@ -445,6 +445,7 @@
     ((nzf_octet<J>(lv[J], kb, dst, o), CSH_SCHED_FENCE()), ...);
     dst[o] = CSH_NZ_END | kb;
 }
+__device__ __forceinline__ static bool nzf_dc_only(const NzFuse &f, const PlaneWork &w) { return f.nz_pool != nullptr && w.nzset != 0xFFFFFFFFu && w.ac_lists != 0u; }
 __device__ __forceinline__ static bool nzf_begin(const NzFuse &f, const PlaneWork &w, NzSet &S) {
     if (!f.nz_pool || w.nzset == 0xFFFFFFFFu) return false;
     S = f.nzsets[w.nzset];
@@ -555,7 +556,7 @@
         load_idct<true>(coef_in + coef_index(gi.tile_base, by * gi.bw + bx, 0), quant[CSH_UNIFORM(im.qt_in[w.comp])], x);
         int vc = gi.comp_w - bx * 8, vr = gi.comp_h - by * 8;
         if (vc < 8 || vr < 8) replicate_edges(x, vc, vr);
-        fdct_quant_store<DERING, true>(x, quant[CSH_UNIFORM(im.qt_out[w.comp])], BlkOut{coef_out, go.tile_base, b, dct_raw, go.tile_base - raw_tile0}, lv, s_dr);
+        fdct_quant_store<DERING, true>(x, quant[CSH_UNIFORM(im.qt_out[w.comp])], BlkOut{coef_out, go.tile_base, b, dct_raw, go.tile_base - raw_tile0, nzf_dc_only(nzf, w)}, lv, s_dr);
         has_raw = dct_raw != nullptr;
     } while (0);
     if (dct_raw) raw_copy_out(dct_raw + raw_index(go.tile_base - raw_tile0, tile * 64), has_raw, s_dr, int(threadIdx.x));
@@ -836,7 +837,7 @@
         const uint2 v = *reinterpret_cast<const uint2 *>(p + size_t(r) * pitch);
         pr[r][0] = bytes_to_halves<0, 1>(v.x); pr[r][2] = bytes_to_halves<2, 3>(v.x); pr[r][1] = bytes_to_halves<3, 2>(v.y); pr[r][3] = bytes_to_halves<1, 0>(v.y);
     }
-    fdct_quant_store_pk<DERING, false>(pr, quant[CSH_UNIFORM(im.qt_out[w.comp])], BlkOut{coef_out, go.tile_base, b, dct_raw, go.tile_base - raw_tile0}, lv, s_dr);
+    fdct_quant_store_pk<DERING, false>(pr, quant[CSH_UNIFORM(im.qt_out[w.comp])], BlkOut{coef_out, go.tile_base, b, dct_raw, go.tile_base - raw_tile0, nzf_dc_only(nzf, w)}, lv, s_dr);
     has_raw = dct_raw != nullptr;
     } while (0);
     if (dct_raw) raw_copy_out(dct_raw + raw_index(go.tile_base - raw_tile0, tile * 64), has_raw, s_dr, int(threadIdx.x));
@@ -960,7 +961,7 @@
                 for (int cc = 0; cc < 4; cc++) pr[r][cc] = pr[r - 1][cc];
             }
     }
-    fdct_quant_store_pk<DERING, false>(pr, quant[CSH_UNIFORM(im.qt_out[w.comp])], BlkOut{coef_out, go.tile_base, b, dct_raw, go.tile_base - raw_tile0}, lv, s_dr);
+    fdct_quant_store_pk<DERING, false>(pr, quant[CSH_UNIFORM(im.qt_out[w.comp])], BlkOut{coef_out, go.tile_base, b, dct_raw, go.tile_base - raw_tile0, nzf_dc_only(nzf, w)}, lv, s_dr);
     has_raw = dct_raw != nullptr;
     } while (0);
     if (dct_raw) raw_copy_out(dct_raw + raw_index(go.tile_base - raw_tile0, tile * 64), has_raw, s_dr, int(threadIdx.x));
diff --git a/caesium-clt_amd/csrc/k_trellis.hip b/caesium-clt_amd/csrc/k_trellis.hip
--- a/caesium-clt_amd/csrc/k_trellis.hip
+++ b/caesium-clt_amd/csrc/k_trellis.hip
@@ -242,7 +242,8 @@
             e = int(Pe & 63u) - 1;
         }
     }
-    int16_t *dst = c.coef + coef_index(g.tile_base, b, 0);
+    const bool to_tile = !(c.ac_lists && w.ac_lists);
+    int16_t *dst = to_tile ? c.coef + coef_index(g.tile_base, b, 0) : nullptr;
     uint32_t *lst = nullptr;
     if (c.nz_pool && w.nzset != 0xFFFFFFFFu) {
         const NzSet &S = c.nzsets[w.nzset];
@@ -266,7 +267,7 @@
                 uint32_t Pe;
                 if (e < CSH_TR_CAP) Pe = L.P[e][tid]; else Pe = CSH_SPILL_LD(sp + ((e - CSH_TR_CAP) * 3u + 2u) * CSH_TR_WGU);
                 const int pos = int((Pe >> 15) & 63u), level = ((kept >> e) & 1ull) ? int((Pe >> 21) & 1023u) : 0;
-                if (!(((kept >> e) & 1ull) && (Pe & 0x4000u))) dst[coef_off(pos)] = int16_t((Pe >> 31) ? -level : level);
+                if (to_tile && !(((kept >> e) & 1ull) && (Pe & 0x4000u))) dst[coef_off(pos)] = int16_t((Pe >> 31) ? -level : level);
                 ent[i] = uint32_t(pos) | ((Pe >> 31) ? 128u : 0u) | (uint32_t(level) << 8) | ((u & 255u) << 23);
             }
         }
diff --git a/caesium-clt_amd/csrc/kernels.h b/caesium-clt_amd/csrc/kernels.h
--- a/caesium-clt_amd/csrc/kernels.h
+++ b/caesium-clt_amd/csrc/kernels.h
@@ -159,6 +159,8 @@
 void launch_list_stats(hipStream_t st, const EncCtx &c);
 void launch_list_refine(hipStream_t st, const EncCtx &c);
 void launch_list_pack(hipStream_t st, const EncCtx &c);
+void launch_nz_to_tiles(hipStream_t st, const NzSet *nzsets, const NzList *nzlists, const uint32_t *nz_pool, const uint32_t *nz_chunk_off, const uint32_t *nz_chunk_cnt,
+                        uint32_t set, uint32_t nchunks, int16_t *coef);
 void launch_reset_works(hipStream_t st, ScanWork *work, int nwork);
 
 #ifndef CSH_TR_WG
@@ -194,6 +196,7 @@
     const NzSet *nzsets;
     const uint32_t *nz_chunk_off, *nz_chunk_cnt;
     const uint16_t *blk_off;
+    uint32_t ac_lists;
 };
 void launch_trellis_sort(hipStream_t st, const TrellisCtx &c);
 void launch_trellis_ac(hipStream_t st, const TrellisCtx &c);
diff --git a/caesium-clt_amd/csrc/pipeline.cpp b/caesium-clt_amd/csrc/pipeline.cpp
--- a/caesium-clt_amd/csrc/pipeline.cpp
+++ b/caesium-clt_amd/csrc/pipeline.cpp
@@ -247,6 +247,7 @@
         t->n_search_extra = b->enc.search ? b->enc.n_gated_runs : 0u;
         t->n_fused_lists = b->enc.last_run_fused;
         t->n_list_refine = b->enc.last_run_refine;
+        t->n_ac_in_lists = b->enc.last_run_ac_lists;
         for (const Item &it : b->items) if (it.image < 0) t->n_failed++;
         for (int i = 0; i < b->nimg; i++) { t->out_bytes += b->out.h_img_size[i]; t->pixels += uint64_t(b->imgs[i].width) * b->imgs[i].height; }
         t->in_bytes = b->dec.bits_pool.size();
@@ -331,6 +332,15 @@
     if (csh_batch_geometry(b, image, comp, which, &bw, &bh, &rbw, &rbh)) return -1;
     const ImgDesc &im = b->imgs[b->items[image].image];
     const CompGeom &g = which ? im.out[comp] : im.in[comp];
+    {
+        const size_t at = size_t(b->items[image].image) * CSH_MAX_COMPS + size_t(comp);
+        const int si = (which && b->enc.last_run_ac_lists && at < b->enc.nzset_of.size()) ? b->enc.nzset_of[at] : -1;
+        if (si >= 0 && size_t(si) < b->enc.nzset_ac_lists.size() && b->enc.nzset_ac_lists[size_t(si)]) {
+            if (hipSetDevice(b->device) != hipSuccess) { csh_set_error("hipSetDevice failed"); return -1; }
+            launch_nz_to_tiles(b->stream, b->enc.d_nzsets.p, b->enc.d_nzlists.p, b->enc.d_nz_pool.p, b->enc.d_nz_chunk_off.p, b->enc.d_nz_chunk_cnt.p, uint32_t(si),
+                               (b->enc.nzsets[size_t(si)].nunits + 255u) / 256u, b->d_coef.p);
+        }
+    }
     std::vector<int16_t> tiles(size_t(g.ntiles) * CSH_TILE_I16);
     if (csh_copy_wait(tiles.data(), b->d_coef.p + size_t(g.tile_base) * CSH_TILE_I16, tiles.size() * 2, hipMemcpyDeviceToHost, b->stream) != hipSuccess) { csh_set_error("D2H failed"); return -1; }
     for (int blk = 0; blk < bw * bh; blk++)
diff --git a/caesium-clt_amd/csrc/types.h b/caesium-clt_amd/csrc/types.h
--- a/caesium-clt_amd/csrc/types.h
+++ b/caesium-clt_amd/csrc/types.h
@@ -121,6 +121,7 @@
     UpDesc up;
     int dn;
     uint32_t nzset;
+    uint32_t ac_lists;
 };
 
 #define CSH_RZ_ANY (-2)
@@ -216,7 +217,7 @@
     uint32_t nunits;
     uint32_t unit_base;
     uint32_t nzset;
-    uint32_t pad[1];
+    uint32_t ac_lists;
 };
 struct TrellisRun { uint32_t work, j, n; };
 
diff --git a/include/caesium_hip.h b/include/caesium_hip.h
--- a/include/caesium_hip.h
+++ b/include/caesium_hip.h
@@ -91,6 +91,7 @@
     uint32_t n_search_extra;
     uint32_t n_fused_lists;
     uint32_t n_list_refine;
+    uint32_t n_ac_in_lists;
 } csh_timing;
 
 int csh_device_count(void);
```

Result: faster. 43880 (median of 6 runs) (+1.5%).
